# VSF1/foo_dsp_resampler

Measured on AMD Instinct MI355X. Metric: Msamples/s, 44.1k->96k float32 'Best' (input channel-samples), higher is better.
Workload: dtype f64; 1 GPU; BASELINE configs[1]: 44.1k->96k 2ch float32 Best; 256 independent 2-channel streams on this GPU, 481689 frames per push, device-resident in/out (RRX_flow_device); streams_per_gpu=256, frames_per_push=481689, channels=2, chain=dft->poly

## Files before the change

### foo_dsp_resampler_amd/csrc/capi.cpp

```cpp
#include "../../include/ratelib_amd.h"

#include "engine.hpp"
#include "finish.hpp"
#include "lpc.hpp"

#include <algorithm>
#include <atomic>
#include <cstdlib>
#include <cstring>
#include <new>
#include <string>
#include <vector>

struct RR_handle_tag {
  rsmp::Engine *eng;
};

namespace {

void (*g_alloc_handler)(void) = nullptr;
int g_initialized = 0;
std::vector<int> g_devices;
std::atomic<unsigned> g_next_device{0};

// ... 167 lines not shown
  }
  if (device < -1) {
    if (handle) *handle = nullptr;
    return RR_INVPARAM;
  }
  return open_common(config, nchannels, nstreams, device, handle, format);
}

int RRX_format(const RR_handle *h) { return h ? h->eng->format() : -1; }

int RRX_push_samples(RR_handle *h, int format, const void *ibuf, size_t in_stride, size_t isamp)
{ return push_host(h, format, ibuf, in_stride, isamp); }

int RRX_pull_samples(RR_handle *h, int format, void *obuf, size_t out_stride, size_t osamp, size_t *ogen)
{ return pull_host(h, format, obuf, out_stride, osamp, ogen); }

int RRX_flow_samples(RR_handle *h, int format, const void *ibuf, size_t in_stride, void *obuf, size_t out_stride, size_t isamp,
                     size_t osamp, size_t *iused, size_t *ogen)
{
  if (h && h->eng->nstreams() == 1) in_stride = isamp, out_stride = osamp;
  return flow_host(h, format, ibuf, in_stride, obuf, out_stride, isamp, osamp, iused, ogen);
}

int RRX_push_device_samples(RR_handle *h, int format, const void *d_ibuf, size_t in_stride, size_t isamp)
{ return push_device(h, format, d_ibuf, in_stride, isamp); }

int RRX_pull_device_samples(RR_handle *h, int format, void *d_obuf, size_t out_stride, size_t osamp, size_t *ogen)
{ return pull_device(h, format, d_obuf, out_stride, osamp, ogen); }

int RRX_flow_device_samples(RR_handle *h, int format, const void *d_ibuf, size_t in_stride, void *d_obuf, size_t out_stride,
                            size_t isamp, size_t osamp, size_t *iused, size_t *ogen)
{ return flow_device(h, format, d_ibuf, in_stride, d_obuf, out_stride, isamp, osamp, iused, ogen); }

int RRX_push_double(RR_handle *h, const double *ibuf, size_t in_stride, size_t isamp)
{ return push_host(h, RRX_FMT_DOUBLE, ibuf, in_stride, isamp); }

int RRX_pull_double(RR_handle *h, double *obuf, size_t out_stride, size_t osamp, size_t *ogen)
{ return pull_host(h, RRX_FMT_DOUBLE, obuf, out_stride, osamp, ogen); }

int RRX_flow_double(RR_handle *h, const double *ibuf, size_t in_stride, double *obuf, size_t out_stride, size_t isamp, size_t osamp,
                    size_t *iused, size_t *ogen)
{
  if (h && h->eng->nstreams() == 1) in_stride = isamp, out_stride = osamp;
  return flow_host(h, RRX_FMT_DOUBLE, ibuf, in_stride, obuf, out_stride, isamp, osamp, iused, ogen);
}

int RRX_push_device_double(RR_handle *h, const double *d_ibuf, size_t in_stride, size_t isamp)
{ return push_device(h, RRX_FMT_DOUBLE, d_ibuf, in_stride, isamp); }

int RRX_pull_device_double(RR_handle *h, double *d_obuf, size_t out_stride, size_t osamp, size_t *ogen)
{ return pull_device(h, RRX_FMT_DOUBLE, d_obuf, out_stride, osamp, ogen); }

int RRX_flow_device_double(RR_handle *h, const double *d_ibuf, size_t in_stride, double *d_obuf, size_t out_stride, size_t isamp,
                           size_t osamp, size_t *iused, size_t *ogen)
{ return flow_device(h, RRX_FMT_DOUBLE, d_ibuf, in_stride, d_obuf, out_stride, isamp, osamp, iused, ogen); }

int RR_push(RR_handle *h, const fb_sample_t *ibuf, size_t isamp) { return push_host(h, RRX_FMT_FLOAT, ibuf, isamp, isamp); }

int RR_pull(RR_handle *h, fb_sample_t *obuf, size_t osamp, size_t *ogen)
{
  const size_t n = h ? (osamp < h->eng->available() ? osamp : h->eng->available()) : 0;
  return pull_host(h, RRX_FMT_FLOAT, obuf, n, osamp, ogen);
}

int RR_flow(RR_handle *h, const fb_sample_t *ibuf, fb_sample_t *obuf, size_t isamp, size_t osamp, size_t *iused, size_t *ogen)
{
  if (h && h->eng->nstreams() != 1) return RR_INVPARAM;
  return flow_host(h, RRX_FMT_FLOAT, ibuf, isamp, obuf, osamp, isamp, osamp, iused, ogen);
}

int RR_drain(RR_handle *h)
{
  if (!h) return RR_NULLHANDLE;
  return guarded(h, [&] { return h->eng->drain(); });
}

void RR_close(RR_handle **h)
{
  if (h == nullptr || *h == nullptr) return;
  delete (*h)->eng;
  delete *h;
  *h = nullptr;
}

const char *RR_strerror(int error)
{
  switch (error) {
    case RR_OK: return "OK";
    case RR_ENOMEM: return "Not enough memory";
    case RR_INTERNAL: return "Internal error";
    case RR_NULLHANDLE: return "NULL handle";
    case RR_RATEERROR: return "Error in rate() functions";
    case RR_EXTUNINIT: return "Externals not initialized";
    default: return "Other error";
  }
}

int RRX_push_device(RR_handle *h, const fb_sample_t *d_ibuf, size_t in_stride, size_t isamp)
{ return push_device(h, RRX_FMT_FLOAT, d_ibuf, in_stride, isamp); }

int RRX_pull_device(RR_handle *h, fb_sample_t *d_obuf, size_t out_stride, size_t osamp, size_t *ogen)
{ return pull_device(h, RRX_FMT_FLOAT, d_obuf, out_stride, osamp, ogen); }

int RRX_flow_device(RR_handle *h, const fb_sample_t *d_ibuf, size_t in_stride, fb_sample_t *d_obuf, size_t out_stride,
                    size_t isamp, size_t osamp, size_t *iused, size_t *ogen)
{ return flow_device(h, RRX_FMT_FLOAT, d_ibuf, in_stride, d_obuf, out_stride, isamp, osamp, iused, ogen); }

int RRX_push_strided(RR_handle *h, const fb_sample_t *ibuf, size_t in_stride, size_t isamp)
{ return push_host(h, RRX_FMT_FLOAT, ibuf, in_stride, isamp); }

int RRX_pull_strided(RR_handle *h, fb_sample_t *obuf, size_t out_stride, size_t osamp, size_t *ogen)
{ return pull_host(h, RRX_FMT_FLOAT, obuf, out_stride, osamp, ogen); }

int RRX_set_stream(RR_handle *h, void *hip_stream)
{
  if (!h) return RR_NULLHANDLE;
  const bool own = hip_stream == RRX_STREAM_OWN;
  return guarded(h, [&] { return h->eng->set_stream(own ? nullptr : static_cast<hipStream_t>(hip_stream), own); });
}

int RRX_sync(RR_handle *h)
{
  if (!h) return RR_NULLHANDLE;
  return guarded(h, [&] { return h->eng->sync(); });
}

int RRX_profile(RR_handle *h, int enable)
{
  if (!h) return RR_NULLHANDLE;
  return guarded(h, [&] { h->eng->set_profiling(enable != 0); return int(RR_OK); });
}

int RRX_profile_read(RR_handle *h, double *hot_ms, long long *hot_launches, double *other_ms, long long *other_launches)
{
  if (!h) return RR_NULLHANDLE;
  return guarded(h, [&] { return h->eng->read_profile(hot_ms, hot_launches, other_ms, other_launches); });
}

int RRX_profile_report(RR_handle *h, char *buf, size_t cap)
{
  if (!h) return -RR_NULLHANDLE;
  if (!buf || !cap) return -RR_INVPARAM;
  std::string s;
  int rc = guarded(h, [&] { return h->eng->read_profile_json(s); });
  if (rc) return -rc;
  size_t n = s.size() < cap - 1 ? s.size() : cap - 1;
  std::memcpy(buf, s.data(), n);
  buf[n] = 0;
  return int(n);
}

void RRX_debug_fail_alloc(int nth) { rsmp::Engine::fail_alloc_after(nth); }

long long RRX_debug_tile_walk(const RRX_walk_geom *g, int k, long long *head, int *slots, size_t cap)
{
  if (!rsmp::knobs().test_hooks || !g || !head || (cap && !slots) || k < 0) return -1;
  if (g->polyL < 1 || g->step < 1 || g->V < 1 || g->n < 1 || g->KS < 1 || g->nsub < 0 || (g->nsub > 0 && g->Vs < 1)) return -1;
  rsmp::FusedPrepArgs pa;
  pa.b_offset = g->b_offset;
  pa.B0 = g->B0;
  pa.at0 = g->at0;
  pa.V = g->V;
  pa.polyL = g->polyL;
  pa.step = g->step;
  pa.n = g->n;
  pa.nblocks = k + 1;
  pa.two_round = g->two_round;
  pa.KS = g->KS;
  pa.qb_max = g->qb_max;
  pa.qb_min = g->qb_min;
  pa.ra_end = g->ra_end;
  pa.rb_start = g->rb_start;
  pa.clip_lo = 0;
  pa.clip_hi = 0x7fffffffffffffffLL;
  pa.nsub = g->nsub;
  pa.Vs = g->Vs;
  return (long long)rsmp::fused_walk_enumerate(pa, k, head, slots, cap);
}

int RRX_lpc_extrapolate_device(int device, void *hip_stream, fb_sample_t *d_data, size_t stream_stride, int nstreams, size_t data_len,
                               int nch, int lpc_order, size_t extra_bkwd, size_t extra_fwd)
{
  if (!d_data || nstreams < 1 || nch < 1 || lpc_order < 1 || lpc_order > rsmp::kLpcMaxOrder || data_len <= size_t(lpc_order)) return RR_INVPARAM;
  if (nstreams > 1 && stream_stride < extra_bkwd + data_len + extra_fwd) return RR_INVPARAM;
  if (device < -1 || (long long)nstreams * nch > 0x7fffffffLL) return RR_INVPARAM;
  if (!g_initialized) return RR_EXTUNINIT;
  if (!extra_bkwd && !extra_fwd) return RR_OK;
  if (device >= 0) {
    int n = 0;
    if (hipGetDeviceCount(&n) != hipSuccess || n < 1) return RR_EXTUNINIT;
    if (device >= n) return RR_INVPARAM;
  }
  if (!rsmp::device_is_gfx950(device)) return RR_EXTUNINIT;
  rsmp::DeviceScope on(device);
  if (!on.ok()) return RR_INTERNAL;
  const hipError_t e = rsmp::launch_lpc_extrapolate(static_cast<hipStream_t>(hip_stream), d_data, stream_stride, nstreams, data_len,
                                                    nch, lpc_order, extra_bkwd, extra_fwd);
  return e == hipSuccess ? RR_OK : RR_INTERNAL;
}

namespace {

int finish_args(int src_format, const void *src, size_t src_stride, int dst_format, void *dst, size_t dst_stride, int nstreams,
                size_t frames, int nch, const double *gain, int dither, unsigned long long seed, unsigned long long first_frame,
                double *peak, unsigned long long *clipped, rsmp::FinishArgs &a)
{
  if (!src || nstreams < 1 || nch < 1) return RR_INVPARAM;
  if (src_format != RRX_FMT_FLOAT && src_format != RRX_FMT_DOUBLE) return RR_INVPARAM;
  if (dst && dst_format != RRX_FMT_S16 && dst_format != RRX_FMT_S24_3 && dst_format != RRX_FMT_S32) return RR_INVPARAM;
  if (nstreams > 1 && (src_stride < frames || (dst && dst_stride < frames))) return RR_INVPARAM;
  if (!dst && !peak && !clipped) return RR_INVPARAM;
  if (first_frame + frames < first_frame) return RR_INVPARAM;
  const size_t most = (~size_t(0) >> 4) / size_t(nch);
  if (frames > most) return RR_INVPARAM;
  if (nstreams > 1 && (src_stride > most / size_t(nstreams) || (dst && dst_stride > most / size_t(nstreams)))) return RR_INVPARAM;
  a.src = src;
  a.dst = dst;
  a.gain = gain;
  a.peak = peak;
  a.clipped = clipped;
  a.src_stride = nstreams > 1 ? (unsigned long long)src_stride * nch : 0;
  a.dst_stride = nstreams > 1 ? (unsigned long long)dst_stride * nch : 0;
  a.n = (unsigned long long)frames * nch;
  a.seed = seed;
  a.first_frame = first_frame;
  a.nstreams = nstreams;
  a.nch = nch;
  a.src_double = src_format == RRX_FMT_DOUBLE;
  a.bits = !dst ? 31 : dst_format == RRX_FMT_S16 ? 15 : dst_format == RRX_FMT_S24_3 ? 23 : 31;
  a.dither = dither != 0;
  return RR_OK;
}

}

int RRX_finish_device(int device, void *hip_stream, int src_format, const void *d_src, size_t src_stride, int dst_format, void *d_dst,
                      size_t dst_stride, int nstreams, size_t frames, int nch, const double *d_gain, int dither, unsigned long long seed,
                      unsigned long long first_frame, double *d_peak, unsigned long long *d_clipped)
{
  rsmp::FinishArgs a;
  const int rc = finish_args(src_format, d_src, src_stride, dst_format, d_dst, dst_stride, nstreams, frames, nch, d_gain, dither, seed,
                             first_frame, d_peak, d_clipped, a);
  if (rc != RR_OK) return rc;
  if (device < -1) return RR_INVPARAM;
  if (!g_initialized) return RR_EXTUNINIT;
  if (!frames) return RR_OK;
  if (device >= 0) {
    int n = 0;
    if (hipGetDeviceCount(&n) != hipSuccess || n < 1) return RR_EXTUNINIT;
    if (device >= n) return RR_INVPARAM;
  }
  if (!rsmp::device_is_gfx950(device)) return RR_EXTUNINIT;
  rsmp::DeviceScope on(device);
  if (!on.ok()) return RR_INTERNAL;
  return rsmp::launch_finish(static_cast<hipStream_t>(hip_stream), a) == hipSuccess ? RR_OK : RR_INTERNAL;
}

int RRX_debug_finish_host(int src_format, const void *src, size_t src_stride, int dst_format, void *dst, size_t dst_stride, int nstreams,
                          size_t frames, int nch, const double *gain, int dither, unsigned long long seed, unsigned long long first_frame,
                          double *peak, unsigned long long *clipped)
{
  if (!rsmp::knobs().test_hooks) return -1;
  rsmp::FinishArgs a;
  const int rc = finish_args(src_format, src, src_stride, dst_format, dst, dst_stride, nstreams, frames, nch, gain, dither, seed,
                             first_frame, peak, clipped, a);
  if (rc != RR_OK) return rc;
  if (frames) rsmp::finish_host(a);
  return RR_OK;
}

int RRX_edge_geometry(size_t in_rate, size_t out_rate, size_t *n_add, size_t *n_drop, size_t *prime_len, size_t *inbuf)
{
  if (!in_rate || !out_rate || !n_add || !n_drop || !prime_len || !inbuf) return RR_INVPARAM;
  size_t a = in_rate, b = out_rate;
  while (b) { const size_t c = a % b; a = b; b = c; }
  const size_t v = a, r1 = in_rate / v, r2 = out_rate / v, z = r1 > r2 ? r1 : r2;
  size_t n = (v + 20 - 1) / 20;
  if (z * n > 8192) n = 8192 / z;
  if (n < 1) n = 1;
  *n_add = r1 * n;
  *n_drop = r2 * n;
  const size_t prime = std::min<size_t>(std::max<size_t>(in_rate / 20, 1024), 16384);
  *prime_len = std::max<size_t>(prime, 2 * rsmp::kLpcMaxOrder + 1);
  *inbuf = std::min<size_t>(std::max<size_t>(in_rate / 10, 2048), 65536);
  return RR_OK;
}

size_t RRX_isamp_max(const RR_handle *h) { return h ? h->eng->isamp_max() : 0; }
size_t RRX_available(const RR_handle *h) { return h ? h->eng->available() : 0; }
int RRX_channels(const RR_handle *h) { return h ? h->eng->nch() : 0; }
int RRX_streams(const RR_handle *h) { return h ? h->eng->nstreams() : 0; }

int RRX_describe_plan(const RR_config *config, char *buf, size_t cap)
{
  if (!config || !buf || !cap) return -RR_INVPARAM;
  rsmp::ChainPlan plan;
  int rc = rsmp::make_plan(to_config(config), plan);
  if (rc) return -rc;
  std::string s = plan.describe();
  size_t n = s.size() < cap - 1 ? s.size() : cap - 1;
  std::memcpy(buf, s.data(), n);
  buf[n] = 0;
  return int(n);
}

int RRX_describe_dispatch(const RR_config *config, int nchannels, char *buf, size_t cap)
{
  if (!config || !buf || !cap || nchannels < 1) return -RR_INVPARAM;
  rsmp::ChainPlan plan;
  int rc = rsmp::make_plan(to_config(config), plan);
  if (rc) return -rc;
  int nsub = 0, vs = 0;
  const bool sub = !plan.stages.empty() && rsmp::split_geometry(plan, nchannels, 0, nsub, vs);
  std::string s = "{\"sub_blocked\": ";
  s += sub ? "true" : "false";
  if (sub) {
    const rsmp::DftFilter &f = plan.dft[plan.stages[0].filt];
    const int V = f.N - (f.num_taps - 1), Pref = f.N / 2;
    const bool two = nsub == 1 && vs > rsmp::kSplitVsMax;
    char tmp[256];
    snprintf(tmp, sizeof tmp, ", \"two_round\": %s, \"nsub\": %d, \"Vs\": %d, \"V\": %d, \"taps\": %d, \"N\": %d, \"Pref\": %d, \"sub_blocks\": [",
             two ? "true" : "false", nsub, vs, V, f.num_taps, f.N, Pref);
    s += tmp;
    for (int i = 0; i < nsub; ++i) {
      const rsmp::SubBlock sb = rsmp::sub_block(i, V, vs, Pref);
      snprintf(tmp, sizeof tmp, "%s{\"off\": %d, \"len\": %d, \"win\": %d, \"shift\": %d}", i ? ", " : "", sb.off, sb.len, sb.win, sb.shift);
      s += tmp;
    }
    s += "]";
  }
// ... 22 lines not shown
```

### foo_dsp_resampler_amd/csrc/engine.cpp

```cpp
#include "engine.hpp"
#include <cstdio>

#include "design.hpp"

#include <algorithm>
#include <atomic>
#include <climits>
#include <cmath>
#include <cstdint>
#include <cstdlib>
#include <cstring>
#include <new>

namespace rsmp {

namespace {

bool pow2_ge2(int x) { return x >= 2 && !(x & (x - 1)); }
bool fdomain_up(int L) { return pow2_ge2(L) && L <= 4; }
int ilog2(long long v) { int l = 0; while ((1LL << l) < v) ++l; return l; }
long long next_pow2(long long v) { long long p = 1; while (p < v) p <<= 1; return p; }

#define HIP_TRY(expr)                                  \
  do {                                                 \
// ... 246 lines not shown
  if (Pref == 4096) {
    if (fused_split_two_supported(V, f.num_taps, mg.KS, mg.qb_max - mg.qb_min) && V >= 2 * p.n) {
      nsub = 1;
      vs = V;
      return true;
    }
  }
  const int vmax = std::min(kSplitVsMax, (2 * 4096 - (f.num_taps - 1)) & ~1);
  if (vmax < 1024) return false;
  const int n_ = (V + vmax - 1) / vmax, v_ = (((V + n_ - 1) / n_) + 1) & ~1;
  if ((n_ - 1) * v_ >= V) return false;
  for (int k = 0; k < n_; ++k) {
    const SubBlock sb = sub_block(k, V, v_, Pref);
    if ((sb.len & 1) || sb.len < 2 * p.n || 2 * sb.shift + sb.len + (f.num_taps - 1) > 8192) return false;
  }
  nsub = n_;
  vs = v_;
  return true;
}

int Engine::init(const Config &cfg, int nch, int nstreams)
{
  int rc = make_plan(cfg, plan_);
  if (rc) return rc;
  nch_ = nch;
  S_ = nstreams;
  C_ = nch * nstreams;

  if (!device_is_gfx950(device_)) return kUninit;
  if ((rc = init_streams()) != kOk) return rc;
  const Knobs &kn = knobs();
  no_side_ = kn.no_side;
  if (kn.stamps) {
    ALLOC_TRY(&stamps_, 16 * sizeof(unsigned long long));
    HIP_TRY(hipMemset(stamps_, 0, 16 * sizeof(unsigned long long)));
  }
  const int ns = int(plan_.stages.size());
  book_.wr.assign(ns + 1, 0);
  book_.rd.assign(ns + 1, 0);
  book_.st.assign(ns, Book::St());
  rings_.assign(ns + 1, Ring());
  big_.assign(ns, BigDft());
  fuse_.assign(ns, Fuse());
  polymf_.assign(ns, PolyMf());
  for (int i = 0; i <= ns; ++i) rings_[i].frames = (i == 0 || i == ns);
  for (int i = 0; i < ns; ++i) {
    const StageSpec &sp = plan_.stages[i];
    book_.wr[i] = sp.preload;
    if (sp.kind == StageKind::Dft) {
      book_.st[i].remL = sp.remL0;
      if ((rc = init_dft_stage(i)) != kOk) return rc;
    } else if (sp.kind == StageKind::Poly) {
      book_.st[i].at = sp.order == 0 ? (sp.at0 >> 32) : sp.at0;
      if (!d_poly_ && (rc = upload(plan_.poly_table, &d_poly_)) != kOk) return rc;
    }
  }
  size_t fused_slab_cap = 0;
  for (int i = 0; i + 1 < ns; ++i)
    if ((rc = init_fused_pair(i, fused_slab_cap)) != kOk) return rc;
  for (int i = 0; i < ns; ++i)
    if ((rc = init_polymf(i)) != kOk) return rc;
  size_slabs(fused_slab_cap);
  for (int i = 0; i <= ns; ++i)
    if ((rc = ensure_ring(i, std::max<long long>(book_.wr[i], 1))) != kOk) return rc;
  HIP_TRY(hipStreamSynchronize(stream_));
  return kOk;
}

int Engine::init_streams()
{
  HIP_TRY(hipStreamCreateWithFlags(&own_, hipStreamNonBlocking));
  stream_ = own_;
  HIP_TRY(hipEventCreateWithFlags(&ev_switch_, hipEventDisableTiming));
  HIP_TRY(hipStreamCreateWithFlags(&side_, hipStreamNonBlocking));
  HIP_TRY(hipEventCreateWithFlags(&ev_fused_, hipEventDisableTiming));
  HIP_TRY(hipEventCreateWithFlags(&ev_seam_[0], hipEventDisableTiming));
  HIP_TRY(hipEventCreateWithFlags(&ev_seam_[1], hipEventDisableTiming));
  return kOk;
}

int Engine::init_dft_stage(int i)
{
  const StageSpec &sp = plan_.stages[i];
  const DftFilter &f = plan_.dft[sp.filt];
  const int Ng = f.N;
  const int log2n = ilog2(Ng);
  const int log2p = fdomain_up(sp.L) ? log2n - ilog2(sp.L) : log2n;
  const int log2nd = sp.step < 0 ? log2n + sp.step : log2n;
  int sub_n = 0, sub_v = 0;
  const bool sub = split_geometry(i, sub_n, sub_v);
  const bool big = log2n > 14 && !sub;
  if (!sub && (big ? !big_dft_supported(log2n, log2p, log2nd) : !dft_shape_supported(log2n, log2p, log2nd))) return kInvParam;
  int rc;
  if (!d_G_[sp.filt] && (rc = upload(component_spectra(f, Ng, 1, sp.L), &d_G_[sp.filt])) != kOk) return rc;
  if (!big && !d_Gr_[sp.filt] && sp.step == 1 && fdomain_up(sp.L) && dftx_supported(log2n, log2p, log2nd) &&
      (rc = upload(component_spectra(f, Ng, sp.L, sp.L), &d_Gr_[sp.filt])) != kOk)
    return rc;
  if (!big) return sub || (twiddles(log2p) && twiddles(log2nd)) ? kOk : kNoMem;
  BigDft &bg = big_[i];
  bg.on = true;
  if (!twiddles(log2p - 4) || !twiddles(log2nd - 4)) return kNoMem;
  std::vector<double2> tw(Ng);
  for (int j = 0; j < Ng; ++j) {
    const long double th = 2.0L * 3.14159265358979323846264338327950288L * (long double)j / (long double)Ng;
    tw[j] = make_double2((double)cosl(th), (double)sinl(th));
  }
  if ((rc = upload(tw, &bg.twN)) != kOk) return rc;
  const int npairs = pair_count(C_, pair_nchs());
  bg.ws_items = int(std::max<long long>(1, std::min<long long>((256LL << 20) / (16LL * Ng), std::max(4 * npairs, 16))));
  ALLOC_TRY(&bg.w1, size_t(bg.ws_items) * (size_t(1) << log2p) * sizeof(double2));
  ALLOC_TRY(&bg.w2, size_t(bg.ws_items) * (size_t(1) << log2nd) * sizeof(double2));
  return kOk;
}

int Engine::init_fused_pair(int i, size_t &slab_cap)
{
  const Knobs &kn = knobs();
  const StageSpec &d = plan_.stages[i], &p = plan_.stages[i + 1];
  if (d.kind != StageKind::Dft || p.kind != StageKind::Poly || p.order != 0 || d.step != 1) return kOk;
  if (!(d.L == 1 || (pow2_ge2(d.L) && d.L <= 4))) return kOk;
  const DftFilter &f = plan_.dft[d.filt];
  const int log2n = ilog2(f.N), log2p = log2n - (d.L == 1 ? 0 : ilog2(d.L));
  const int G = 2, pstep = int(p.step64 >> 32), at0 = int(p.at0 >> 32);
  int dmax = 0;
  const int NG = (p.L + G - 1) / G;
  for (int m = 0; m < NG; ++m) {
    const long long a0 = at0 + (long long)(G * m) * pstep, a1 = at0 + (long long)std::min(G * m + G - 1, p.L - 1) * pstep;
    dmax = std::max(dmax, int(a1 / p.L - a0 / p.L));
  }
  const int max_seam = int(((long long)(p.n - 1) * p.L + pstep - 1) / pstep) + 1;
  int split_nsub = 0, split_vs = 0;
  split_geometry(i, split_nsub, split_vs);
  const bool split = split_nsub > 0;
  const int threads = split ? 256 : f.N / 16;
  if (!split && (NG > threads || !fused_shape_supported(log2n, log2p, p.n, p.n + dmax, max_seam))) return kOk;
  if (kn.no_fuse) return kOk;
  Fuse &fu = fuse_[i];
  fu.on = true;
  fu.nsub = split_nsub;
  fu.Vs = split_vs;
  int rc;
  if (split) {
    if (!twiddles(12)) return kNoMem;
    if ((rc = upload(component_spectra(f, 8192, 2, d.L), &fu.Gs)) != kOk) return rc;
  }
  fu.span = p.n + dmax;
  fu.NG = NG;
  fu.KC = split ? 1 : threads / NG;
  fu.blk_cap = 64;
  while (fu.blk_cap < kFusedMaxBlocks && double(C_ + 1) * double(4 * fu.blk_cap) * 512 <= kn.seam_ring_mb * 1048576.0) fu.blk_cap *= 2;
  while (fu.blk_cap < 8 * split_nsub) fu.blk_cap *= 2;
  fu.slots = 2 * fu.blk_cap;
  ALLOC_TRY(&fu.blk_dev, size_t(2 * fu.blk_cap) * sizeof(FusedBlock));
  const size_t bytes = size_t(C_ + 1) * fu.slots * 2 * 32 * sizeof(double);
  ALLOC_TRY(&fu.seam, bytes);
  HIP_TRY(hipMemset(fu.seam, 0, bytes));
  const int V = f.N - (f.num_taps - 1);
  const int Kmax = int(((long long)V * p.L / pstep + p.L - 1) / p.L) + 2;
  fu.kper = (Kmax + fu.KC - 1) / fu.KC;
  if (!split && (rc = upload(vector_tiles(p, G, NG, fu.KC, threads, plan_.poly_table), &fu.cft)) != kOk) return rc;
  const MfGeom mg = mf_geom(p);
  bool lanes_spread = true;
  if (kn.spread_vector)
    for (int j1 = 0; j1 < 4; ++j1)
      for (int j2 = j1 + 1; j2 < 4; ++j2)
        if (((j2 - j1) * pstep) % 16 == 0) lanes_spread = false;
  const bool rounds_ok = (mg.qb_max - mg.qb_min) + 4 * mg.KS + 4 <= (kFusedSA - kFusedSB0) * 256 + 32 && Kmax <= 32 && p.L >= 64 && lanes_spread;
  if (split || (!kn.no_mfma && fused_mfma_supported(log2n, log2p, mg.KS) && rounds_ok)) {
    const MfOperands op = mf_operands(mg, p, plan_.poly_table);
    if ((rc = upload(op.cfm, &fu.cfm)) != kOk || (rc = upload(op.cfm2, &fu.cfm2)) != kOk || (rc = upload(op.qtab, &fu.qtab)) != kOk)
      return rc;
    fu.NGRP = mg.NGRP;
    fu.KS = mg.KS;
    fu.qb_max = mg.qb_max;
    fu.qb_min = mg.qb_min;
  }
  const size_t per_launch = size_t(fu.blk_cap / std::max(1, fu.nsub) - 2) * size_t((V - d.remL0 + d.L - 1) / d.L);
  double ahead = 1;
  for (int k = 0; k < i; ++k) ahead *= plan_.stages[k].kind == StageKind::Half ? 0.5 : plan_.stages[k].out_in_ratio;
  const size_t cap = size_t(double(per_launch) / std::max(ahead, 1e-9));
  slab_cap = slab_cap ? std::min(slab_cap, cap) : cap;
  return kOk;
}

int Engine::init_polymf(int i)
{
  const Knobs &kn = knobs();
  const StageSpec &p = plan_.stages[i];
  if (p.kind != StageKind::Poly || p.order != 0 || (i > 0 && fuse_[i - 1].on) || p.L < 64) return kOk;
  if (kn.no_mfma || kn.no_polymf) return kOk;
  const int pstep = int(p.step64 >> 32);
  const MfGeom mg = mf_geom(p);
  if (!polymf_supported(mg.KS)) return kOk;
  int Vt = 2048;
  while (Vt > 256 && ((long long)Vt * p.L / pstep + p.L - 1) / p.L + 2 > 30) Vt -= 256;
  if (((long long)Vt * p.L / pstep + p.L - 1) / p.L + 2 > 30) return kOk;
  const MfOperands op = mf_operands(mg, p, plan_.poly_table);
  PolyMf &pm = polymf_[i];
  int rc;
  if ((rc = upload(op.cfm, &pm.cfm)) != kOk || (rc = upload(op.qtab, &pm.qtab)) != kOk) return rc;
  pm.KS = mg.KS;
  pm.NGRP = mg.NGRP;
  pm.Vt = Vt;
  pm.blk_cap = 4096;
  ALLOC_TRY(&pm.blk, size_t(pm.blk_cap) * sizeof(FusedBlock));
  return kOk;
}

void Engine::size_slabs(size_t fused_slab_cap)
{
  const int ns = int(plan_.stages.size());
  double bytes_per_in_frame = 0, rate = 1;
  for (int i = 0; i < ns; ++i) {
    const StageSpec &sp = plan_.stages[i];
    if (sp.kind == StageKind::Dft) rate *= sp.step > 0 ? double(sp.L) / sp.step : double(sp.L) / double(1 << -sp.step);
    else if (sp.kind == StageKind::Poly) rate *= sp.out_in_ratio;
    else rate *= 0.5;
    if (i + 1 < ns && !fuse_[i].on) bytes_per_in_frame += rate * 8.0 * C_;
  }
  const double budget = knobs().slab_mb * 1024 * 1024;
  slab_frames_ = bytes_per_in_frame > 0 ? size_t(budget / bytes_per_in_frame) : plan_.isamp_max;
  slab_frames_ = std::max<size_t>(slab_frames_, 8192);
  slab_frames_ = std::min<size_t>(slab_frames_, std::max<size_t>(plan_.isamp_max, 1));
  if (fused_slab_cap) slab_frames_ = std::max<size_t>(1024, std::min(slab_frames_, fused_slab_cap));
}

void Engine::set_profiling(bool on)
{
  profiling_ = on;
  for (ProfRec &r : prof_) {
    (void)hipEventDestroy(r.e0);
    (void)hipEventDestroy(r.e1);
  }
  prof_.clear();
}

int Engine::prof_begin(bool hot, const char *name)
{
  if (!profiling_) return -1;
  ProfRec r;
  r.hot = hot;
  r.name = name;
  if (hipEventCreate(&r.e0) != hipSuccess || hipEventCreate(&r.e1) != hipSuccess) return -1;
  (void)hipEventRecord(r.e0, stream_);
  prof_.push_back(r);
  return int(prof_.size()) - 1;
}

void Engine::prof_end(int idx)
{
  if (idx >= 0) (void)hipEventRecord(prof_[idx].e1, stream_);
}

int Engine::read_profile(double *hot_ms, long long *hot_launches, double *other_ms, long long *other_launches)
{
  HIP_TRY(hipStreamSynchronize(stream_));
  double h = 0, o = 0;
  long long hn = 0, on = 0;
  for (ProfRec &r : prof_) {
    float ms = 0;
    if (hipEventElapsedTime(&ms, r.e0, r.e1) == hipSuccess) {
      if (r.hot) { h += ms; ++hn; } else { o += ms; ++on; }
    }
    (void)hipEventDestroy(r.e0);
    (void)hipEventDestroy(r.e1);
  }
  prof_.clear();
  if (hot_ms) *hot_ms = h;
  if (hot_launches) *hot_launches = hn;
  if (other_ms) *other_ms = o;
  if (other_launches) *other_launches = on;
  return kOk;
}

int Engine::read_profile_json(std::string &out)
{
  HIP_TRY(hipStreamSynchronize(stream_));
  struct Agg { const char *name; bool hot; long long n; double ms; };
  std::vector<Agg> agg;
  for (ProfRec &r : prof_) {
    float ms = 0;
    if (hipEventElapsedTime(&ms, r.e0, r.e1) == hipSuccess) {
      Agg *a = nullptr;
      for (Agg &x : agg)
        if (std::strcmp(x.name, r.name) == 0 && x.hot == r.hot) a = &x;
      if (!a) {
        agg.push_back(Agg{r.name, r.hot, 0, 0.0});
        a = &agg.back();
      }
      a->n += 1;
      a->ms += ms;
    }
    (void)hipEventDestroy(r.e0);
    (void)hipEventDestroy(r.e1);
  }
  prof_.clear();
  out = "[";
  char buf[64];
  for (size_t i = 0; i < agg.size(); ++i) {
    out += i ? ", {" : "{";
    out += "\"kernel\": \"";
    out += agg[i].name;
    snprintf(buf, sizeof buf, "\", \"hot\": %d, \"launches\": %lld, \"ms\": %.6f}", agg[i].hot ? 1 : 0, agg[i].n, agg[i].ms);
    out += buf;
  }
  out += "]";
  return kOk;
}

int Engine::join_side()
{
  if (!side_pending_) return kOk;
  HIP_TRY(hipStreamWaitEvent(stream_, ev_seam_[(seam_launches_ - 1) & 1], 0));
  side_pending_ = false;
  return kOk;
}

int Engine::pinned_reserve(Pinned &b, size_t bytes)
{
  if (!b.done) HIP_TRY(hipEventCreateWithFlags(&b.done, hipEventDisableTiming));
  if (b.bytes >= bytes) return kOk;
  if (b.p) {
    HIP_TRY(hipStreamSynchronize(stream_));
    (void)hipHostFree(b.p);
  }
  b.p = nullptr;
  b.bytes = 0;
  size_t want = 16384;
  while (want < bytes) want <<= 1;
  void *p = nullptr;
  if (hipHostMalloc(&p, want, hipHostMallocDefault) != hipSuccess) {
    (void)hipGetLastError();
    return kNoMem;
  }
  b.p = p;
  b.bytes = want;
  return kOk;
}

void Engine::pinned_free(Pinned &b)
{
  if (b.p) (void)hipHostFree(b.p);
  if (b.done) (void)hipEventDestroy(b.done);
  b = Pinned();
}

void Engine::free_garbage()
{
  for (void *p : garbage_) (void)hipFree(p);
  garbage_.clear();
}

Engine::~Engine()
{
  DeviceScope on(device_);
  (void)hipStreamSynchronize(stream_);
  if (own_ && own_ != stream_) (void)hipStreamSynchronize(own_);
  if (side_) (void)hipStreamSynchronize(side_);
  free_garbage();
  for (Ring &r : rings_) if (r.buf) (void)hipFree(r.buf);
  for (double2 *&g : d_G_) if (g) (void)hipFree(g);
  for (double2 *&g : d_Gr_) if (g) (void)hipFree(g);
  if (d_poly_) (void)hipFree(d_poly_);
  for (double2 *&t : d_tw_) if (t) (void)hipFree(t);
  for (double2 *&t : d_tw8_) if (t) (void)hipFree(t);
  set_profiling(false);
  if (d_stage_) (void)hipFree(d_stage_);
  pinned_free(pin_in_[0]);
  pinned_free(pin_in_[1]);
  pinned_free(pin_out_);
  pinned_free(pin_mir_);
  if (stamps_) {
    unsigned long long h[16] = {};
    if (hipMemcpy(h, stamps_, sizeof(h), hipMemcpyDeviceToHost) == hipSuccess && h[7])
      fprintf(stderr, "RSMP_STAMPS workgroups %llu  avg cycles: load %.0f  fwd %.0f  mul %.0f  inv %.0f  cf+smp %.0f  polyA %.0f  poly(B) %.0f  total %.0f\n",
              h[7], double(h[0]) / h[7], double(h[1]) / h[7], double(h[2]) / h[7], double(h[3]) / h[7], double(h[4]) / h[7],
              double(h[6]) / h[7], double(h[5]) / h[7], double(h[0] + h[1] + h[2] + h[3] + h[4] + h[5] + h[6]) / h[7]);
    (void)hipFree(stamps_);
  }
  for (Fuse &f : fuse_) {
    if (f.seam) (void)hipFree(f.seam);
    if (f.cft) (void)hipFree(f.cft);
    if (f.cfm) (void)hipFree(f.cfm);
    if (f.qtab) (void)hipFree(f.qtab);
    if (f.cfm2) (void)hipFree(f.cfm2);
    if (f.Gs) (void)hipFree(f.Gs);
    if (f.blk_dev) (void)hipFree(f.blk_dev);
  }
  for (BigDft &b : big_) {
    if (b.twN) (void)hipFree(b.twN);
    if (b.w1) (void)hipFree(b.w1);
    if (b.w2) (void)hipFree(b.w2);
  }
  for (PolyMf &m : polymf_) {
    if (m.cfm) (void)hipFree(m.cfm);
    if (m.qtab) (void)hipFree(m.qtab);
    if (m.blk) (void)hipFree(m.blk);
  }
  if (side_) (void)hipStreamDestroy(side_);
  if (ev_fused_) (void)hipEventDestroy(ev_fused_);
  for (hipEvent_t &e : ev_seam_) if (e) (void)hipEventDestroy(e);
  if (ev_switch_) (void)hipEventDestroy(ev_switch_);
  if (own_) (void)hipStreamDestroy(own_);
}

int Engine::set_stream(hipStream_t s, bool own)
{
  hipStream_t next = own ? own_ : s;
  if (next == stream_) return kOk;
  { int rcj = join_side(); if (rcj) return rcj; }
  HIP_TRY(hipEventRecord(ev_switch_, stream_));
  HIP_TRY(hipStreamWaitEvent(next, ev_switch_, 0));
  stream_ = next;
  return kOk;
}

int Engine::sync()
{
  HIP_TRY(hipStreamSynchronize(stream_));
  free_garbage();
  return kOk;
}

AnyView Engine::view(int f, const ExtIn *ein, const ExtOut *eout) const
{
  const Ring &r = rings_[f];
  AnyView v = {};
  if (!r.frames) {
    v.kind = kRingF64;
    v.d.ring = static_cast<double *>(r.buf);
    v.d.mask = r.cap - 1;
    v.d.chan_stride = r.cap;
    return v;
  }
  v.kind = fk_;
  v.f.ring = r.buf;
  v.f.ring_mask = r.cap - 1;
  v.f.ring_stream_stride = r.cap * nch_;
  v.f.nch = nch_;
  if (ein && ein->ptr) {
    v.f.ext = const_cast<void *>(ein->ptr);
    v.f.ext_begin = ein->begin;
    v.f.ext_end = ein->end;
    v.f.ext_stream_stride = ein->stride_elems;
  } else if (eout && eout->ptr) {
    v.f.ext = eout->ptr;
    v.f.ext_begin = eout->begin;
    v.f.ext_end = eout->end;
    v.f.ext_stream_stride = eout->stride_elems;
  }
  return v;
}

int Engine::ensure_ring(int f, long long live_needed)
{
  Ring &r = rings_[f];
  if (r.buf && r.cap >= live_needed) return kOk;
  { int rcj = join_side(); if (rcj) return rcj; }
  const long long cap = next_pow2(std::max<long long>({live_needed, r.cap * 2, 4096}));
  const size_t bytes = r.frames ? size_t(cap) * nch_ * S_ * size_t(eb_) : size_t(cap) * C_ * sizeof(double);
  void *nb = nullptr;
  ALLOC_TRY(&nb, bytes);
  HIP_TRY(hipMemsetAsync(nb, 0, bytes, stream_));
  if (r.buf) {
    Ring old = r;
    r.buf = nb;
    r.cap = cap;
    const long long a0 = book_.rd[f], a1 = book_.wr[f];
    const AnyView dst = view(f);
    AnyView src = dst;
    if (r.frames) {
      src.f.ring = old.buf;
      src.f.ring_mask = old.cap - 1;
      src.f.ring_stream_stride = old.cap * nch_;
    } else {
      src.d.ring = static_cast<double *>(old.buf);
      src.d.mask = old.cap - 1;
      src.d.chan_stride = old.cap;
    }
    HIP_TRY(launch_copy(src, dst, a0, a1, C_, stream_));
    garbage_.push_back(old.buf);
  } else {
    r.buf = nb;
    r.cap = cap;
  }
  return kOk;
}

void Engine::note_input(Book &b, size_t n) const
{
  b.samples_in += n;
  while (b.samples_in > plan_.cfg.in_rate && b.samples_out > plan_.cfg.out_rate) {
    b.samples_in -= plan_.cfg.in_rate;
    b.samples_out -= plan_.cfg.out_rate;
  }
}

#define RSMP_STAGE_LOCALS(ps, i)                                                                                   \
  Book &b = (ps).b;                                                                                                \
  const bool launch = (ps).launch;                                                                                 \
  const ExtIn &ein = (ps).ein;                                                                                     \
  const ExtOut &eout = (ps).eout;                                                                                  \
  const int ns = int(plan_.stages.size());                                                                         \
  const StageSpec &sp = plan_.stages[i];                                                                           \
  Book::St &st = b.st[i];                                                                                          \
  long long &rd = b.rd[i];                                                                                         \
  long long &wro = b.wr[(i) + 1];                                                                                  \
  const long long occ = b.wr[i] - rd;                                                                              \
                                              \
  const bool src_frames = (i) == 0, dst_frames = (i) + 1 == ns;                                                    \
  const long long rd_before = rd, wro_before = wro;                                                                \
  const long long out_offset = (i) + 1 < ns ? plan_.stages[(i) + 1].preload : -b.trimmed;                          \
  Pending &pend = (ps).pend;                                                                                       \
                                      \
  auto dst_need = [&](long long wr_after) {                                                                        \
    if (dst_frames && eout.ptr) return std::max<long long>(0, wr_after - std::max(eout.end, b.rd[(i) + 1]));      \
    return wr_after - b.rd[(i) + 1];                                                                               \
  };                                                                                                               \
  (void)rd_before; (void)wro_before; (void)out_offset; (void)occ; (void)src_frames; (void)dst_frames;             \
  (void)launch; (void)ein; (void)pend; (void)st; (void)dst_need

int Engine::advance(Book &b, size_t n_new, bool launch, const ExtIn &ein, const ExtOut &eout, bool more_slabs)
{
  note_input(b, n_new);
  b.wr[0] += (long long)n_new;
  Pass ps{b, launch, ein, eout, more_slabs, Pending()};
  for (int i = 0; i < int(plan_.stages.size()); ++i) {
    const StageKind kind = plan_.stages[i].kind;
    const int rc = kind == StageKind::Dft ? advance_dft(ps, i) : kind == StageKind::Poly ? advance_poly(ps, i) : advance_half(ps, i);
    if (rc) return rc;
  }
  return kOk;
}

int Engine::advance_dft(Pass &ps, int i)
{
  RSMP_STAGE_LOCALS(ps, i);
  DftArgs &pend_args = pend.args;
  int &pend_log2n = pend.log2n, &pend_log2p = pend.log2p;
  const DftFilter &f = plan_.dft[sp.filt];
// ... 39 lines not shown
    if (!sub && !big && log2p >= 6 && log2p <= 13 && !a.tw_fwd8) return kNoMem;
    a.tw_inv8 = (!sub && !big && log2nd >= 6 && log2nd <= 12) ? twiddles8(log2nd) : nullptr;
    if (!sub && !big && log2nd >= 6 && log2nd <= 12 && !a.tw_inv8) return kNoMem;
    a.B0 = B0;
    a.out_offset = out_offset;
    a.nblocks = nblocks;
    a.C = C_;
    a.L = L;
    a.c0 = pow2_ge2(L) ? 0 : sp.remL0;
    a.V = Vg;
    a.Vout = sp.step < 0 ? Ng - ((((1 << -sp.step) - 1) * Ng + ov) >> -sp.step) : Vg;
    a.q = (Vg - sp.remL0 + L - 1) / L;
    a.M = sp.step > 1 ? sp.step : 1;
    a.hp = 0;
    a.nchs = pair_nchs();
    a.in_limit = 0x7fffffffffffffffLL;
    a.clip_lo = -0x7fffffffffffffffLL;
    a.clip_hi = 0x7fffffffffffffffLL;
    a.nsub = a.Vs = a.Pref = a.two = 0;
    a.Bref0 = 0;
    if (big) {
      const BigDft &bg = big_[i];
      BigDftArgs ba;
      ba.d = a;
      ba.twN = bg.twN;
      ba.w1 = bg.w1;
      ba.w2 = bg.w2;
      ba.log2n = log2n;
      ba.log2mp = log2p - 4;
      ba.log2md = log2nd - 4;
      ba.fdomain_in = (log2p < log2n || L == 1) ? 1 : 0;
      ba.item0 = 0;
      const int pi = prof_begin(true, "rsmp::big_cols_fwd_kernel + big_rows_kernel + big_cols_inv_kernel");
      HIP_TRY(launch_dft_big(view(i, &ein), view(i + 1, nullptr, &eout), ba, bg.ws_items, stream_));
      prof_end(pi);
    } else
    if (fused) {
      pend.B0 = B0;
      pend.nblocks = nblocks;
      pend_args = a;
      pend_log2n = log2n;
      pend_log2p = log2p;
    } else if (a.Gr && sp.step == 1 && fdomain_up(L) && dftx_supported(log2n, log2p, log2nd)) {
      const int pi = prof_begin(true);
      const char *kn = nullptr;
      HIP_TRY(launch_dftx(log2n, view(i, &ein), view(i + 1, nullptr, &eout), a, stream_, &kn));
      prof_name(pi, kn);
      prof_end(pi);
    } else {
    const int pi = prof_begin(true);
    const char *kn = nullptr;
    HIP_TRY(launch_dft(log2n, log2p, log2nd, view(i, &ein), view(i + 1, nullptr, &eout), a, stream_, &kn));
    prof_name(pi, kn);
    prof_end(pi);
    }
  }
  return kOk;
}

int Engine::advance_poly(Pass &ps, int i)
{
  RSMP_STAGE_LOCALS(ps, i);
  const long long num_in = std::max<long long>(0, occ - sp.pre_post);
  long long count = 0, at_end = st.at;
  const long long step = sp.order == 0 ? (sp.step64 >> 32) : sp.step64;
  const long long lim = sp.order == 0 ? num_in * sp.L : (num_in << 32);
  if (st.at < lim) count = (lim - st.at + step - 1) / step;
  at_end = st.at + count * step;
  const bool fused = i > 0 && fuse_[i - 1].on;
  if (launch && fused) {
    if ((count != 0) != (pend.nblocks != 0)) return kInternal;
    if (pend.nblocks) {
      const int rc = launch_fused_pair(ps, i, count, step);
      if (rc) return rc;
    }
  } else if (launch && count && polymf_[i].cfm) {
    const int rc = launch_polymf_stage(ps, i, count, step);
    if (rc) return rc;
  } else if (launch && count) {
    const int rc = launch_poly_stage(ps, i, count, step);
    if (rc) return rc;
  }
  if (sp.order == 0) {
    rd += at_end / sp.L;
    st.at = at_end % sp.L;
  } else {
    rd += at_end >> 32;
    st.at = at_end & 0xffffffffLL;
  }
  wro += count;
  return kOk;
}

int Engine::launch_fused_pair(Pass &ps, int i, long long count, long long step)
{
  RSMP_STAGE_LOCALS(ps, i);
  const bool more_slabs = ps.more_slabs;
  DftArgs &pend_args = pend.args;
  const int pend_log2n = pend.log2n, pend_log2p = pend.log2p;
  int rc = ensure_ring(i + 1, dst_need(wro + count));
  if (rc) return rc;
  const Fuse &fu = fuse_[i - 1];
  FusedArgs fa;
  fa.d = pend_args;
  fa.tab = d_poly_;
  fa.seam = fu.seam;
  fa.cft = fu.cft;
  fa.at0 = sp.at0 >> 32;
  fa.b_offset = sp.preload;
  fa.out_offset2 = out_offset;
  fa.seam_mask = fu.slots - 1;
  fa.n = sp.n;
  fa.polyL = sp.L;
  fa.step = int(step);
  fa.span = fu.span;
  fa.NG = fu.NG;
  fa.KC = fu.KC;
  fa.kper = fu.kper;
  fa.cfm = fu.cfm;
  fa.qtab = fu.qtab;
  fa.cfm2 = fu.cfm2;
  fa.NGRP = fu.NGRP;
  fa.KS = fu.KS;
  fa.stamps = stamps_;
  const bool split = fu.nsub > 0;
  const int ntab = split ? pend.nblocks * fu.nsub : pend.nblocks;
  if (ntab > fu.blk_cap) return kInternal;
  FusedPrepArgs pa;
  pa.b_offset = fa.b_offset;
  pa.B0 = pend.B0;
  pa.at0 = fa.at0;
  pa.V = fa.d.V;
  pa.polyL = sp.L;
  pa.step = int(step);
  pa.n = sp.n;
  pa.nblocks = ntab;
  pa.nsub = fu.nsub;
  pa.Vs = fu.Vs;
  const bool split_two = split && fu.nsub == 1 && fu.Vs > kSplitVsMax;
  pa.two_round = fu.cfm != nullptr && (!split || split_two);
  pa.ra_end = split_two ? kSplitRaEnd : 0;
  pa.rb_start = split_two ? kSplitRbStart : 0;
  pa.KS = fu.KS;
  pa.qb_max = fu.qb_max;
  pa.qb_min = fu.qb_min;
  pa.clip_lo = 0;
  pa.clip_hi = 0x7fffffffffffffffLL;
  if (!split)
    for (int k : {0, pend.nblocks - 1})
      if (fused_block_info(pa, k).K > (fu.cfm ? 32 : fu.KC * fu.kper)) return kInternal;
  const bool seam_on_side = more_slabs && !(profiling_ || !dst_frames || no_side_);
  if (seam_launches_ >= 2) HIP_TRY(hipStreamWaitEvent(stream_, ev_seam_[seam_launches_ & 1], 0));
  FusedBlock *const blk_half = fu.blk_dev + size_t(seam_launches_ & 1) * fu.blk_cap;
  { const int pp = prof_begin(false, "rsmp::fused_prep_kernel"); HIP_TRY(launch_fused_prep(pa, blk_half, stream_)); prof_end(pp); }
  fa.blk = blk_half;
  const long long endnum = (b.wr[i] - sp.n + 1) * sp.L - fa.at0;
  if (wro - out_offset + count != (endnum <= 0 ? 0 : (endnum + step - 1) / step)) return kInternal;
  const bool in_frames = i - 1 == 0;
  int f0 = 0, f1 = 0;
  FastIo io = {};
  io.dio = fk_ - kFramesF32;
  const uintptr_t amask = 2 * uintptr_t(eb_) - 1;
  auto io_in = [&] {
    io.in = ein.ptr;
    io.in_ring = rings_[0].buf;
    io.in_ring_mask = rings_[0].cap - 1;
    io.in_ring_stream_stride = rings_[0].cap * nch_;
    io.in_abs0 = ein.begin;
    io.in_stream_stride = ein.stride_elems;
    io.nch = nch_;
  };
  auto io_out64 = [&] {
    io.out64 = static_cast<double *>(rings_[i + 1].buf);
    io.out64_mask = rings_[i + 1].cap - 1;
    io.out64_chan_stride = rings_[i + 1].cap;
  };
  if (split) {
    if (!in_frames || (nch_ & 1) || !ein.ptr || (ein.stride_elems & 1)) return kInternal;
    io_in();
    io.in_unaligned = (reinterpret_cast<uintptr_t>(ein.ptr) & amask) ? 1 : 0;
    int omode = 1;
    if (!dst_frames)
      io_out64();
    else {
      const bool ext_ok = eout.ptr && !(eout.stride_elems & 1);
      const bool all_inside = ext_ok && wro >= eout.begin && wro + count <= eout.end;
      omode = (all_inside && !(reinterpret_cast<uintptr_t>(eout.ptr) & amask)) ? 0 : 2;
      io.out = ext_ok ? eout.ptr : nullptr;
      io.out_abs0 = ext_ok ? eout.begin : 0;
      io.out_end = ext_ok ? eout.end : 0;
      io.out_stream_stride = ext_ok ? eout.stride_elems : 0;
      io.out_unaligned = (ext_ok && (reinterpret_cast<uintptr_t>(eout.ptr) & amask)) ? 1 : 0;
      io.out_ring = rings_[i + 1].buf;
      io.out_ring_mask = rings_[i + 1].cap - 1;
      io.out_ring_stream_stride = rings_[i + 1].cap * nch_;
      if (eout.ptr && !ext_ok) return kInternal;
      if (omode == 2 && !io.out_ring) return kInternal;
    }
    FusedArgs fr = fa;
    fr.d.G = fu.Gs;
    fr.d.tw_fwd = fr.d.tw_inv = twiddles(12);
    if (!fr.d.tw_fwd) return kNoMem;
    fr.d.nsub = fu.nsub;
    fr.d.Vs = fu.Vs;
    fr.d.two = split_two ? 1 : 0;
    fr.d.Pref = 1 << pend_log2p;
    fr.d.Bref0 = pend.B0;
    fr.d.B0 = pend.B0 * fu.nsub;
    fr.d.nblocks = ntab;
    fa = fr;
    const int pi = prof_begin(true);
    const char *kn = nullptr;
    HIP_TRY(launch_fused_split(omode, fr, io, stream_, &kn));
    prof_name(pi, kn);
    prof_end(pi);
  } else if (fu.cfm && in_frames && dst_frames && !(nch_ & 1) && ein.ptr && eout.ptr && fused_fast_supported(pend_log2n, pend_log2p, fu.KS) &&
             !(reinterpret_cast<uintptr_t>(ein.ptr) & amask) && !(reinterpret_cast<uintptr_t>(eout.ptr) & amask) &&
             !(ein.stride_elems & 1) && !(eout.stride_elems & 1)) {
    const long long P = 1LL << pend_log2p, q = fa.d.q;
    const long long hi = (ein.end - P) >= 0 ? (ein.end - P) / q - pend.B0 + 1 : 0;
    f0 = 0;
    f1 = int(std::min<long long>(pend.nblocks, hi));
    while (f0 < f1) {
      const FusedBlock b0 = fused_block_info(pa, f0), b1 = fused_block_info(pa, f1 - 1);
      if (out_offset + b0.i_lo < eout.begin) { ++f0; continue; }
      if (out_offset + b1.i_lo + b1.cnt > eout.end) { --f1; continue; }
      break;
    }
    if (f0 >= f1) f0 = f1 = 0;
    io_in();
    io.out = eout.ptr;
    io.out_abs0 = eout.begin;
    io.out_stream_stride = eout.stride_elems;
  } else if (fu.cfm && in_frames && !dst_frames && !(nch_ & 1) && ein.ptr && fused_fast_supported(pend_log2n, pend_log2p, fu.KS) &&
             !(reinterpret_cast<uintptr_t>(ein.ptr) & amask) && !(ein.stride_elems & 1)) {
    const long long P = 1LL << pend_log2p, q = fa.d.q;
    const long long hi = (ein.end - P) >= 0 ? (ein.end - P) / q - pend.B0 + 1 : 0;
    f0 = 0;
    f1 = int(std::max<long long>(0, std::min<long long>(pend.nblocks, hi)));
    io_in();
    io_out64();
  }
  auto launch_range = [&](int b0, int b1, bool fast) -> int {
    if (b0 >= b1) return kOk;
    FusedArgs fr = fa;
    fr.d.B0 = fa.d.B0 + b0;
    fr.d.nblocks = b1 - b0;
    fr.blk = fa.blk + b0;
    const int pi = prof_begin(true);
    const char *kn = nullptr;
    if (fast) HIP_TRY(launch_fused_fast(pend_log2p, fr, io, stream_, &kn));
    else
      HIP_TRY(launch_fused(pend_log2n, pend_log2p, view(i - 1, &ein), view(i + 1, nullptr, &eout), fr, stream_, &kn));
    prof_name(pi, kn);
    prof_end(pi);
    return kOk;
  };
  if (!split) {
    { int rl = launch_range(0, f0, false); if (rl) return rl; }
    { int rl = launch_range(f0, f1, true); if (rl) return rl; }
    { int rl = launch_range(f1, pend.nblocks, false); if (rl) return rl; }
  }
  if (!seam_on_side) {
    { int rcj = join_side(); if (rcj) return rcj; }
    const int ps = prof_begin(false, "rsmp::seam_kernel");
    HIP_TRY(launch_seam(view(i + 1, nullptr, &eout), fa, stream_));
    prof_end(ps);
  } else {
    HIP_TRY(hipEventRecord(ev_fused_, stream_));
    HIP_TRY(hipStreamWaitEvent(side_, ev_fused_, 0));
    HIP_TRY(launch_seam(view(i + 1, nullptr, &eout), fa, side_));
    HIP_TRY(hipEventRecord(ev_seam_[seam_launches_ & 1], side_));
    ++seam_launches_;
    side_pending_ = true;
  }
  return kOk;
}

int Engine::launch_polymf_stage(Pass &ps, int i, long long count, long long step)
{
  RSMP_STAGE_LOCALS(ps, i);
  int rc = ensure_ring(i + 1, dst_need(wro + count));
  if (rc) return rc;
  const PolyMf &pm = polymf_[i];
  const long long at0 = sp.at0 >> 32, i_begin = wro_before - out_offset, i_end = i_begin + count;
  const long long q_first = (at0 + i_begin * step) / sp.L, q_last = (at0 + (i_end - 1) * step) / sp.L;
  for (long long t0 = q_first / pm.Vt, t_end = q_last / pm.Vt + 1; t0 < t_end; t0 += pm.blk_cap) {
    FusedPrepArgs pa;
    pa.b_offset = 0;
    pa.B0 = t0;
    pa.at0 = at0;
    pa.V = pm.Vt;
    pa.polyL = sp.L;
    pa.step = int(step);
    pa.n = 1;
    pa.nblocks = int(std::min<long long>(pm.blk_cap, t_end - t0));
    pa.two_round = 0;
    pa.ra_end = pa.rb_start = 0;
    pa.nsub = pa.Vs = 0;
    pa.KS = pm.KS;
    pa.qb_max = 0;
    pa.qb_min = 0;
    pa.clip_lo = i_begin;
    pa.clip_hi = i_end;
    for (int k : {0, pa.nblocks - 1})
      if (fused_block_info(pa, k).K > 32) return kInternal;
    { const int pp = prof_begin(false, "rsmp::fused_prep_kernel"); HIP_TRY(launch_fused_prep(pa, pm.blk, stream_)); prof_end(pp); }
    PolyMfArgs a;
    a.cfm = pm.cfm;
    a.qtab = pm.qtab;
    a.blk = pm.blk;
    a.B0 = t0;
    a.at0 = at0;
    a.out_offset = out_offset;
    a.in_limit = b.wr[i];
    a.nblocks = pa.nblocks;
    a.C = C_;
    a.Vt = pm.Vt;
    a.n = sp.n;
    a.polyL = sp.L;
    a.step = int(step);
    a.NGRP = pm.NGRP;
    a.nchs = pair_nchs();
    const int pi = prof_begin(false);
    const char *kn = nullptr;
    HIP_TRY(launch_polymf(pm.KS, view(i, &ein), view(i + 1, nullptr, &eout), a, stream_, &kn));
    prof_name(pi, kn);
    prof_end(pi);
  }
  return kOk;
}

int Engine::launch_poly_stage(Pass &ps, int i, long long count, long long step)
{
  RSMP_STAGE_LOCALS(ps, i);
  int rc = ensure_ring(i + 1, dst_need(wro + count));
  if (rc) return rc;
  PolyArgs a;
  a.tab = d_poly_;
  a.rd = rd_before;
  a.at = st.at;
  a.step = step;
  a.out_abs = wro_before;
  a.count = count;
  a.C = C_;
  a.n = sp.n;
  a.L = sp.L;
  a.phase_bits = sp.phase_bits;
  const double in_per_out = sp.order == 0 ? double(step) / sp.L : double(step) / 4294967296.0;
  const size_t tab_bytes = sp.order == 0 ? size_t(sp.L) * sp.n * 8 : 0;
  const bool tab_lds = sp.order == 0 && tab_bytes <= 40 * 1024;
  const double lds_for_window = tab_lds ? double(64 * 1024 - 16) - double(tab_bytes) : 48.0 * 1024;
  int tile = 2048;
  while (tile > 256 && ((tile * in_per_out + sp.n + 4) * 8 > lds_for_window ||
                        (sp.order == 0 && double(tile + 256) * double(step) >= 2147483648.0)))
    tile >>= 1;
  if (sp.order == 0 && double(tile + 256) * double(step) >= 2147483648.0) return kInternal;
  a.tile = tile;
  a.win = (int(tile * in_per_out) + sp.n + 4 + 1) & ~1;
  a.tab_lds = tab_lds;
  a.coop = sp.order >= 1 && sp.n % 8 == 0 && !knobs().no_polycoop;
  a.shared_rows = 0;
  if (sp.order >= 1 && sp.n <= 32 && !knobs().no_polyi) {
    const double wl = 128 * in_per_out + sp.n + 4;
    if ((128.0 * sp.n + 16.0 * (wl + 1)) * 8 <= 150.0 * 1024) {
      a.shared_rows = 1;
      a.tile = 128;
      a.win = int(wl) | 1;
    }
  }
  const int pi = prof_begin(false);
  const char *kn = nullptr;
  HIP_TRY(launch_poly(sp.order, view(i, &ein), view(i + 1, nullptr, &eout), a, stream_, &kn));
  prof_name(pi, kn);
  prof_end(pi);
  return kOk;
}

int Engine::advance_half(Pass &ps, int i)
{
  RSMP_STAGE_LOCALS(ps, i);
  const long long avail = std::max<long long>(0, occ - sp.pre_post);
  const long long num_out = (avail + 1) / 2;
  if (launch && num_out) {
    int rc = ensure_ring(i + 1, dst_need(wro + num_out));
    if (rc) return rc;
    HalfArgs a;
    a.rd = rd_before;
    a.out_abs = wro_before;
    a.count = num_out;
    a.C = C_;
    a.ncoef = sp.hb_n;
    a.pre = sp.pre;
    for (int k = 0; k < 13; ++k) a.coef[k] = k < sp.hb_n ? sp.hb[k] : 0.0;
    const int pi = prof_begin(false);
    const char *kn = nullptr;
    HIP_TRY(launch_half(view(i, &ein), view(i + 1, nullptr, &eout), a, stream_, &kn));
    prof_name(pi, kn);
    prof_end(pi);
  }
  if (2 * num_out <= occ) rd += 2 * num_out;
// ... 336 lines not shown
```

### foo_dsp_resampler_amd/csrc/engine.hpp

```cpp
#pragma once
#include "kernels.hpp"
#include "plan.hpp"

#include <hip/hip_runtime.h>
#include <cstddef>
#include <cstdint>
#include <string>
#include <vector>

namespace rsmp {

enum { kOk = 0, kNoMem = 1, kInternal = 2, kNullHandle = 3, kRateError = 4, kUninit = 5, kInvParam = 6 };

struct Book {
  std::vector<long long> wr, rd;
  struct St { long long B = 0; int remL = 0, remM = 0; long long at = 0; };
  std::vector<St> st;
  size_t samples_in = 0, samples_out = 0;
  long long trimmed = 0;
};

bool split_geometry(const ChainPlan &plan, int nch, int i, int &nsub, int &vs);

class DeviceScope {
public:
  explicit DeviceScope(int device)
  {
    if (hipGetDevice(&prev_) != hipSuccess) prev_ = -1;
    if (device >= 0 && device != prev_) ok_ = hipSetDevice(device) == hipSuccess, switched_ = ok_;
  }
  ~DeviceScope() { if (switched_ && prev_ >= 0) (void)hipSetDevice(prev_); }
  DeviceScope(const DeviceScope &) = delete;
  DeviceScope &operator=(const DeviceScope &) = delete;
  bool ok() const { return ok_; }
private:
  int prev_ = -1;
  bool ok_ = true, switched_ = false;
};

class Engine {
public:
  static int create(const Config &cfg, int nch, int nstreams, int device, Engine **out, int fmt = 0);
  ~Engine();

  int device() const { return device_; }
  int format() const { return fmt_; }

  const ChainPlan &plan() const { return plan_; }
  int nch() const { return nch_; }
  int nstreams() const { return S_; }
  int pair_nchs() const { return (S_ > 1 && (nch_ & 1)) ? nch_ : 0; }
  size_t isamp_max() const { return plan_.isamp_max; }
  size_t available() const { return size_t(book_.wr.back() - book_.rd.back()); }

  int set_stream(hipStream_t s, bool own = false);
  hipStream_t stream() const { return stream_; }
  int sync();
  static void fail_alloc_after(int n);

  int push_host(const void *ibuf, size_t stream_stride, size_t isamp);
  int pull_host(void *obuf, size_t stream_stride, size_t osamp, size_t *ogen);
  int flow_host(const void *ibuf, size_t in_stride, void *obuf, size_t out_stride, size_t isamp, size_t osamp, size_t *iused,
                size_t *ogen);
  int push_device(const void *ibuf, size_t stream_stride, size_t isamp);
  int pull_device(void *obuf, size_t stream_stride, size_t osamp, size_t *ogen);
  int flow_device(const void *ibuf, size_t in_stride, void *obuf, size_t out_stride, size_t isamp, size_t osamp, size_t *iused,
                  size_t *ogen);
  int drain();

  void set_profiling(bool on);
  int read_profile(double *hot_ms, long long *hot_launches, double *other_ms, long long *other_launches);
  int read_profile_json(std::string &out);

private:
  Engine() = default;
  int init(const Config &cfg, int nch, int nstreams);
  int init_streams();
  int init_dft_stage(int i);
  int init_fused_pair(int i, size_t &slab_cap);
  int init_polymf(int i);
  void size_slabs(size_t fused_slab_cap);
  int fmt_ = 0, eb_ = 4, fk_ = kFramesF32;
  size_t frame_bytes() const { return size_t(nch_) * size_t(eb_); }
  static const void *at_bytes(const void *p, size_t bytes) { return static_cast<const char *>(p) + bytes; }
  static void *at_bytes(void *p, size_t bytes) { return static_cast<char *>(p) + bytes; }

  struct Ring {
    void *buf = nullptr;
    long long cap = 0;
    bool frames = false;
  };
  struct ExtIn { const void *ptr = nullptr; long long begin = 0, end = 0, stride_elems = 0; };
  struct ExtOut { void *ptr = nullptr; long long begin = 0, end = 0, stride_elems = 0; };

  int feed(const void *d_in, size_t stride_frames, size_t isamp, void *d_out, size_t out_stride, size_t out_cap,
           size_t *direct_out, bool keep_direct = false);
  int feed_impl(const void *d_in, size_t stride_frames, size_t isamp, void *d_out, size_t out_stride, size_t out_cap,
                size_t *direct_out, bool keep_direct);
  int advance(Book &b, size_t n_new, bool launch, const ExtIn &ein, const ExtOut &eout, bool more_slabs = false);
  struct Pending { long long B0 = 0; int nblocks = 0; DftArgs args = {}; int log2n = 0, log2p = 0; };
  struct Pass { Book &b; bool launch; const ExtIn &ein; const ExtOut &eout; bool more_slabs; Pending pend; };
  int advance_dft(Pass &ps, int i);
  int advance_poly(Pass &ps, int i);
  int advance_half(Pass &ps, int i);
  int launch_fused_pair(Pass &ps, int i, long long count, long long step);
  bool split_geometry(int i, int &nsub, int &vs) const;
  int launch_polymf_stage(Pass &ps, int i, long long count, long long step);
  int launch_poly_stage(Pass &ps, int i, long long count, long long step);
  int ensure_ring(int f, long long live_needed);
  int copy_out(void *dst, size_t stride_frames, size_t frames, bool to_host);
  AnyView view(int f, const ExtIn *ein = nullptr, const ExtOut *eout = nullptr) const;
  void note_input(Book &b, size_t n) const;
  template <class T> int upload(const std::vector<T> &src, T **dst);
  const double2 *twiddles(int log2m);
  const double2 *twiddles8(int log2m);
  void free_garbage();

  ChainPlan plan_;
  int nch_ = 0, S_ = 0, C_ = 0;
  int device_ = 0;
  hipStream_t stream_ = nullptr;
  hipStream_t own_ = nullptr;
  hipEvent_t ev_switch_ = nullptr;
  bool poisoned_ = false;
  int fail(int rc) { if (rc != kOk) poisoned_ = true; return rc; }
  int dev_alloc(void **p, size_t bytes);
  hipStream_t side_ = nullptr;
  hipEvent_t ev_fused_ = nullptr, ev_seam_[2] = {nullptr, nullptr};
  long long seam_launches_ = 0;
  bool side_pending_ = false;
  int join_side();
  Book book_;
  std::vector<Ring> rings_;
  std::vector<void *> garbage_;
  double2 *d_G_[2] = {nullptr, nullptr};
  double2 *d_Gr_[2] = {nullptr, nullptr};
  double *d_poly_ = nullptr;
  double2 *d_tw_[20] = {};
  double2 *d_tw8_[20] = {};
  struct BigDft { bool on = false; double2 *twN = nullptr, *w1 = nullptr, *w2 = nullptr; int ws_items = 0; };
  std::vector<BigDft> big_;
  struct Fuse { bool on = false; int span = 0, NG = 0, KC = 0, kper = 0; double *seam = nullptr; double *cft = nullptr; int slots = 0;
                double *cfm = nullptr; int NGRP = 0, KS = 0, qb_max = 0, qb_min = 0; int *qtab = nullptr; double2 *cfm2 = nullptr;
                FusedBlock *blk_dev = nullptr; int blk_cap = 0;
                int nsub = 0, Vs = 0; double2 *Gs = nullptr; };
  std::vector<Fuse> fuse_;
  struct PolyMf { double *cfm = nullptr; int *qtab = nullptr; FusedBlock *blk = nullptr; int KS = 0, NGRP = 0, Vt = 0, blk_cap = 0; };
  std::vector<PolyMf> polymf_;
  struct ProfRec { hipEvent_t e0, e1; bool hot; const char *name; };
  std::vector<ProfRec> prof_;
  bool profiling_ = false;
  int prof_begin(bool hot, const char *name = "");
  void prof_name(int idx, const char *name) { if (idx >= 0 && name) prof_[idx].name = name; }
  void prof_end(int idx);
  bool no_side_ = false;
  unsigned long long *stamps_ = nullptr;
  void *d_stage_ = nullptr;
  size_t stage_bytes_ = 0;
  struct Pinned { void *p = nullptr; size_t bytes = 0; hipEvent_t done = nullptr; bool pending = false; };
  Pinned pin_in_[2], pin_out_;
  int pin_k_ = 0;
  static constexpr size_t kPinnedMaxBytes = size_t(64) << 20;
  static constexpr size_t kZeroCopyMaxBytes = size_t(1) << 20;
  Pinned pin_mir_;
  long long mir_begin_ = 0, mir_end_ = 0;
  size_t mir_stride_ = 0;
  int spill_mirror();
  int pinned_reserve(Pinned &b, size_t bytes);
  void pinned_free(Pinned &b);
  size_t slab_frames_ = 0;
};

bool device_is_gfx950(int device = -1);

}
```

### foo_dsp_resampler_amd/csrc/fused.hip

```cpp
#include "fft_device.hpp"
#include "fifo_device.hpp"
#include "kernels.hpp"

#include <algorithm>
#include <type_traits>
#include <atomic>
#include <cstdlib>
#include <cstdio>


namespace rsmp {

constexpr int kPad = 32;
constexpr int kSpanMax = 32;
constexpr int kSA = kFusedSA, kSB0 = kFusedSB0;

template <int LOG2N, int LOG2P, int G, int SPAN, bool MF>
__global__ __launch_bounds__((1 << LOG2N) / 16, MF ? kFusedWaves : 2) void fused_kernel(AnyView in, AnyView out, FusedArgs a)
{
  constexpr int N = 1 << LOG2N, P = 1 << LOG2P;
  constexpr int T = N / 16, TF = P / 16;
  extern __shared__ __attribute__((aligned(16))) double lds[];

  const int tid = threadIdx.x;
// ... 335 lines not shown
      const int kr0 = kc * kper, kr1 = min(kr0 + kper, fb.K);

      bool ofast = false;
      float *obase = nullptr;
      int ostride = 1;
      const PairSpan o64 = out.kind >= kFramesF64 ? pair_span(out, pair, hasb, a.out_offset2 + fb.i_lo, fb.cnt, ca)
                                                    : PairSpan{0, nullptr, 1, nullptr, nullptr, hasb};
      {
        const long long o0 = a.out_offset2 + fb.i_lo, o1 = o0 + fb.cnt;
        if (out.kind == kFramesF32 && hasb && !(out.f.nch & 1)) {
          const int hp = out.f.nch >> 1, strm = pair / hp, pin = pair - strm * hp;
          ostride = hp;
          if (out.f.ext && o0 >= out.f.ext_begin && o1 <= out.f.ext_end) {
            obase = static_cast<float *>(out.f.ext) + strm * out.f.ext_stream_stride + (o0 - out.f.ext_begin) * out.f.nch + 2 * pin;
            ofast = true;
          } else if ((!out.f.ext || o0 >= out.f.ext_end || o1 <= out.f.ext_begin) &&
                     (o0 & out.f.ring_mask) + (o1 - o0) <= out.f.ring_mask + 1) {
            obase = static_cast<float *>(out.f.ring) + strm * out.f.ring_stream_stride + (o0 & out.f.ring_mask) * out.f.nch + 2 * pin;
            ofast = true;
          }
          ofast = ofast && (reinterpret_cast<unsigned long long>(obase) & 7) == 0;
        }
      }

      for (int kr = kr0; kr < kr1; ++kr) {
        const int ib = kr * pl + r0;
        bool ok[G], any = false;
#pragma unroll
        for (int g = 0; g < G; ++g) {
          ok[g] = rv[g] && ib + g >= fb.irel_lo && ib + g < irel_hi;
          any = any || ok[g];
        }
        if (!any) continue;
        const int li = qr0 + kr * step + fb.base_li;
        const double2 *xw = smp + li;
        double accA[G], accB[G];
#pragma unroll
        for (int g = 0; g < G; ++g) accA[g] = accB[g] = 0.0;
#pragma unroll
        for (int mm = 0; mm < SPAN; ++mm) {
          const double2 xv = xw[mm];
#pragma unroll
          for (int g = 0; g < G; ++g) {
            accA[g] = fma(cf[g][mm], xv.x, accA[g]);
            accB[g] = fma(cf[g][mm], xv.y, accB[g]);
          }
        }
        const int orel = ib - fb.irel_lo;
        if (ofast) {
          float2 *o2 = reinterpret_cast<float2 *>(obase) + orel * ostride;
          if (G == 2 && ostride == 1 && ok[0] && ok[1] && (reinterpret_cast<unsigned long long>(o2) & 15) == 0) {
            *reinterpret_cast<float4 *>(o2) = make_float4((float)accA[0], (float)accB[0], (float)accA[1], (float)accB[1]);
          } else {
#pragma unroll
            for (int g = 0; g < G; ++g)
              if (ok[g]) o2[g * ostride] = make_float2((float)accA[g], (float)accB[g]);
          }
        } else if (o64.kind == 3) {
#pragma unroll
          for (int g = 0; g < G; ++g)
            if (ok[g]) o64.d2[(orel + g) * o64.fstride] = make_double2(accA[g], accB[g]);
        } else if (o64.kind >= 4) {
#pragma unroll
          for (int g = 0; g < G; ++g)
            if (ok[g]) o64.puti(orel + g, accA[g], accB[g]);
        } else {
          const ChanRef oa = chan_ref(out, ca), ob = chan_ref(out, hasb ? cb : ca);
          const long long oabs = a.out_offset2 + fb.i_lo + orel;
#pragma unroll
          for (int g = 0; g < G; ++g)
            if (ok[g]) {
              fifo_put(oa, oabs + g, accA[g]);
              if (hasb) fifo_put(ob, oabs + g, accB[g]);
            }
        }
      }
    }
    RSMP_STAMP(5)
    if (stamping && tid == 0) atomicAdd(a.stamps + 7, 1ull);
  }
#undef RSMP_STAMP
}

constexpr int kSeamC = 64, kSeamWin = 2 * 31 + 3, kSeamOut = 64;
__global__ __launch_bounds__(256) void seam_kernel(AnyView out, FusedArgs a)
{
  __shared__ double win[kSeamC][kSeamWin];
  __shared__ double cfs[kSeamOut][32];
  __shared__ int qs[kSeamOut];
  const int bl = blockIdx.x, c0 = blockIdx.y * kSeamC, tid = threadIdx.x;
  const long long B = a.d.B0 + bl;
  const int nm1 = a.n - 1, pl = a.polyL, step = a.step, n = a.n;
  const int nc = min(kSeamC, a.d.C - c0);
  const FusedBlock fb = a.blk[bl];
  const int cnt = min((int)(fb.i_lo - fb.seam_i0), kSeamOut);
  {
    const int k = tid & 63;
    const double *const tails = a.seam + ((long long)((int)((B - 1) & a.seam_mask) * (a.d.C + 1) + c0) * 2 + 1) * 32;
    const double *const heads = a.seam + ((long long)((int)(B & a.seam_mask) * (a.d.C + 1) + c0) * 2) * 32;
    const bool wk = k < 2 * nm1;
    const double *const src = k < nm1 ? tails + k : heads + (min(k, 2 * nm1 - 1) - nm1);
    const bool zero = k < nm1 && B == 0;
    double tw[kSeamC / 4];
#pragma unroll
    for (int i = 0; i < kSeamC / 4; ++i) tw[i] = src[min((tid >> 6) + 4 * i, nc - 1) * 64];
    const int j = min(tid & 31, n - 1);
    double t[kSeamOut / 8];
    int q[kSeamOut / 8];
#pragma unroll
    for (int i = 0; i < kSeamOut / 8; ++i) {
      t[i] = 0.0;
      q[i] = 0;
      if (8 * i < cnt) {
        const int u = min((tid >> 5) + 8 * i, cnt - 1);
        const unsigned tc = (unsigned)fb.seam_ph0 + (unsigned)u * (unsigned)step;
        const unsigned qq = tc / (unsigned)pl, ph = tc - qq * (unsigned)pl;
        q[i] = fb.seam_q0 + (int)qq;
        t[i] = a.tab[(long long)ph * n + j];
      }
    }
    if (wk) {
#pragma unroll
      for (int i = 0; i < kSeamC / 4; ++i) {
        const int cl = (tid >> 6) + 4 * i;
        if (cl < nc) win[cl][k] = zero ? 0.0 : tw[i];
      }
    }
#pragma unroll
    for (int i = 0; i < kSeamOut / 8; ++i) {
      const int u = (tid >> 5) + 8 * i;
      if (u < cnt) {
        if ((tid & 31) < n) cfs[u][j] = t[i];
        if ((tid & 31) == 0) qs[u] = q[i];
      }
    }
  }
  __syncthreads();
  {
    const int cl = tid & 63;
    if (cl < nc) {
      const ChanRef oc = chan_ref(out, c0 + cl);
      for (int u = tid >> 6; u < cnt; u += 4) {
        const double *x = win[cl] + qs[u];
        const double *cf = cfs[u];
        double sum = 0.0;
#pragma unroll 8
        for (int j = 0; j < n; ++j) sum = fma(cf[j], x[j], sum);
        fifo_put(oc, a.out_offset2 + fb.seam_i0 + u, sum);
      }
    }
  }
}

__global__ __launch_bounds__(256) void fused_prep_kernel(FusedPrepArgs p, FusedBlock *out)
{
  const int k = blockIdx.x * 256 + threadIdx.x;
  if (k < p.nblocks) out[k] = fused_block_info(p, k);
}

hipError_t launch_fused_prep(const FusedPrepArgs &p, FusedBlock *out, hipStream_t st)
{
  hipLaunchKernelGGL(fused_prep_kernel, dim3((p.nblocks + 255) / 256), dim3(256), 0, st, p, out);
  return hipGetLastError();
}

template <int LOG2N, int LOG2P, int G, int SPAN, bool MF>
static hipError_t launch_fused_t(const AnyView &in, const AnyView &out, const FusedArgs &a, hipStream_t st)
{
  constexpr int N = 1 << LOG2N;
  const size_t lds_pad = knobs().lds_pad;
  size_t lds_bytes = 8 * size_t(fft_lds_doubles(LOG2N));
  if (MF) {
    lds_bytes = 8 * size_t(fft_lds_doubles_halves(LOG2N));
    if (LOG2P < LOG2N) lds_bytes = std::max(lds_bytes, 8 * size_t(std::max(fft_lds_doubles(LOG2P), fft8_lds_doubles(LOG2P))));
    lds_bytes = std::max(lds_bytes, size_t(kPad + kSA * (N / 16) + kPad) * 16);
  }
  lds_bytes += lds_pad;
  static DynLdsOnce attr;
  static std::atomic<bool> occ_printed{false};
  if (hipError_t e = attr.set(reinterpret_cast<const void *>(&fused_kernel<LOG2N, LOG2P, G, SPAN, MF>), int(lds_bytes)); e != hipSuccess) return e;
  {
    if (knobs().occ && !occ_printed.exchange(true)) {
      int nb = -1;
      hipError_t eo = hipOccupancyMaxActiveBlocksPerMultiprocessor(&nb, reinterpret_cast<const void *>(&fused_kernel<LOG2N, LOG2P, G, SPAN, MF>), N / 16, lds_bytes);
      fprintf(stderr, "RSMP_OCC lds %zu blocks/CU %d (%s)\n", lds_bytes, nb, hipGetErrorString(eo));
    }
  }
  FusedArgs b = a;
  b.d.hp = frame_pairs(in, out, a.d.C);
  b.d.npairs = pair_count(a.d.C, a.d.nchs);
  b.d.pps_magic = pair_magic(a.d.C, a.d.nchs);
  dim3 grid(item_grid(a.d.nblocks, b.d.npairs, b.d.hp)), block(N / 16);
  hipLaunchKernelGGL((fused_kernel<LOG2N, LOG2P, G, SPAN, MF>), grid, block, lds_bytes, st, in, out, b);
  return hipGetLastError();
}

hipError_t launch_seam(const AnyView &out, const FusedArgs &a, hipStream_t st)
{
  dim3 sgrid(a.d.nblocks, (a.d.C + kSeamC - 1) / kSeamC), sblock(256);
  hipLaunchKernelGGL(seam_kernel, sgrid, sblock, 0, st, out, a);
  return hipGetLastError();
}

bool fused_mfma_supported(int log2n, int log2p, int ksteps)
{
  return log2n == 12 && (log2p == 11 || log2p == 12) && (ksteps == 7 || ksteps == 8);
}

bool fused_shape_supported(int log2n, int log2p, int n, int span, int max_seam_outputs)
{
  if (log2n < 11 || log2n > 13) return false;
  if (log2p > log2n || log2p < log2n - 2) return false;
  return n >= 4 && n <= 32 && span <= kSpanMax && max_seam_outputs <= 64;
}

#define RSMP_FUSED_CASE(n, p)                                                     \
  if (log2n == n && log2p == p) {                                                 \
    if (kname) *kname = "rsmp::fused_kernel<" #n ", " #p ", 2, 32, false>";       \
    return launch_fused_t<n, p, 2, kSpanMax, false>(in, out, a, st);              \
  }
#define RSMP_FUSED_EXACT(n, p, sp)                                                \
  if (log2n == n && log2p == p && a.span == sp) {                                 \
    if (kname) *kname = "rsmp::fused_kernel<" #n ", " #p ", 2, " #sp ", false>";  \
    return launch_fused_t<n, p, 2, sp, false>(in, out, a, st);                    \
  }
#define RSMP_FUSED_MF(n, p, ks)                                                   \
  if (log2n == n && log2p == p && a.KS == ks) {                                   \
    if (kname) *kname = "rsmp::fused_kernel<" #n ", " #p ", 2, " #ks ", true>";   \
    return launch_fused_t<n, p, 2, ks, true>(in, out, a, st);                     \
  }

hipError_t launch_fused(int log2n, int log2p, const AnyView &in, const AnyView &out, const FusedArgs &a, hipStream_t st,
                        const char **kname)
{
  if (a.cfm) {
    RSMP_FUSED_MF(12, 11, 7) RSMP_FUSED_MF(12, 12, 7) RSMP_FUSED_MF(12, 11, 8) RSMP_FUSED_MF(12, 12, 8)
    return hipErrorInvalidValue;
  }
  RSMP_FUSED_EXACT(12, 11, 25) RSMP_FUSED_EXACT(12, 11, 26) RSMP_FUSED_EXACT(12, 12, 26) RSMP_FUSED_EXACT(12, 12, 27)
  RSMP_FUSED_CASE(11, 11) RSMP_FUSED_CASE(11, 10) RSMP_FUSED_CASE(11, 9)
  RSMP_FUSED_CASE(12, 12) RSMP_FUSED_CASE(12, 11) RSMP_FUSED_CASE(12, 10)
  RSMP_FUSED_CASE(13, 13) RSMP_FUSED_CASE(13, 12) RSMP_FUSED_CASE(13, 11)
  return hipErrorInvalidValue;
}

}
```

### foo_dsp_resampler_amd/csrc/fused_fast.hip

```cpp
#include "fft_device.hpp"
#include "fifo_device.hpp"
#include "kernels.hpp"

#include <algorithm>
#include <atomic>
#include <cstdlib>
#include <cstdio>
#include <type_traits>

namespace rsmp {

namespace {
typedef unsigned int rsmp_v2u __attribute__((ext_vector_type(2)));
typedef unsigned int rsmp_v4u __attribute__((ext_vector_type(4)));
template <typename E> struct Frame;
template <> struct Frame<float> {
  typedef float2 P;
  static __device__ __forceinline__ double in(float s) { return (double)s; }
  static __device__ __forceinline__ float out(double y) { return (float)y; }
};
template <> struct Frame<double> {
  typedef double2 P;
  static __device__ __forceinline__ double in(double s) { return s; }
  static __device__ __forceinline__ double out(double y) { return y; }
};
template <> struct Frame<short> {
  typedef short2 P;
  static __device__ __forceinline__ double in(short s) { return pcm_in(s); }
  static __device__ __forceinline__ short out(double y) { return pcm_out16(y); }
};
template <> struct Frame<int> {
  typedef int2 P;
  static __device__ __forceinline__ double in(int s) { return pcm_in(s); }
  static __device__ __forceinline__ int out(double y) { return pcm_out32(y); }
};
__device__ __forceinline__ double2 load_g(const double2 *p) { return *p; }
constexpr int kPad = 32;
constexpr int kSA = kFusedSA, kSB0 = kFusedSB0;
}

template <int LOG2P, int KS, bool OUT64, bool SPLIT, bool OGEN, bool TWO = false, typename E = float>
__device__ __forceinline__ void fused_fast_body(const FusedArgs &a, const FastIo &io)
{
  typedef Frame<E> Fr;
  typedef typename Fr::P E2;
  const E *const io_in = static_cast<const E *>(io.in), *const io_in_ring = static_cast<const E *>(io.in_ring);
  E *const io_out = static_cast<E *>(io.out), *const io_out_ring = static_cast<E *>(io.out_ring);
  static_assert(!TWO || SPLIT, "two rounds from registers: sub-blocked form only");
  static_assert(!SPLIT || LOG2P == 12, "sub-blocked form: 4096-point components");
  static_assert(!OGEN || (SPLIT && !OUT64), "generic float output exists for the sub-blocked form only");
  constexpr int LOG2N = 12, N = 1 << LOG2N, P = 1 << LOG2P;
  constexpr int T = N / 16, TF = P / 16;
  extern __shared__ __attribute__((aligned(16))) double lds[];

  const int tid = threadIdx.x;
  const int npairs = a.d.C >> 1;
  int bl, pair;
  if (!item_map(blockIdx.x, a.d.nblocks, npairs, a.d.hp, bl, pair)) return;
  const long long B = a.d.B0 + bl;
  const int hp = io.nch >> 1, strm = pair / hp, pin = pair - strm * hp;
  SubBlock sb = {0, 0, 0, 0};
  long long e0_split = 0;
  if constexpr (SPLIT) {
    const int kr = bl / a.d.nsub;
    sb = sub_block(bl - kr * a.d.nsub, a.d.V, a.d.Vs, a.d.Pref);
    e0_split = (a.d.Bref0 + kr) * a.d.q + sb.win;
  }
  const int V = SPLIT ? sb.len : a.d.V;
  const bool fwd_active = tid < TF;
  const double2 *__restrict__ Gp = a.d.G;
  double2 *smp = reinterpret_cast<double2 *>(lds) + kPad;
  const int nm1 = a.n - 1;

#ifdef RSMP_STAMPS_BUILD
  const bool stamping = a.stamps && (blockIdx.x & 63) == 5;
  unsigned long long tstamp = stamping ? __builtin_readcyclecounter() : 0;
#define RSMP_STAMP(slot)                                          \
  if (stamping) {                                                  \
    const unsigned long long now = __builtin_readcyclecounter();  \
    if (tid == 0) atomicAdd(a.stamps + (slot), now - tstamp);      \
    tstamp = now;                                                  \
  }
#else
#define RSMP_STAMP(slot)
#endif

  constexpr bool FWD8 = LOG2P == LOG2N - 1;
  constexpr int NLD = FWD8 ? 8 : 16, TL = FWD8 ? T : TF;
  c64 v[16];
  c64 u8[8];
  c64 z0[SPLIT ? 16 : 1];
  double2 wf[FWD8 ? fft8_tw_regs(LOG2P) : 1];
  if constexpr (FWD8) fft8_tw_load<LOG2P>(wf, tid, a.d.tw_fwd8);
  {
    const long long e0 = SPLIT ? e0_split : B * a.d.q;
    const bool ld_active = FWD8 || fwd_active;
    if (SPLIT && io.in_unaligned) {
      const E *pe = io_in + strm * io.in_stream_stride + 2 * pin, *pr = io_in_ring + strm * io.in_ring_stream_stride + 2 * pin;
#pragma unroll
      for (int s = 0; s < NLD; ++s) {
        const long long e = e0 + tid + s * TL;
        const E *f = e >= io.in_abs0 ? pe + (e - io.in_abs0) * io.nch : pr + (e & io.in_ring_mask) * io.nch;
        v[s] = {Fr::in(f[0]), Fr::in(f[1])};
      }
    } else
    if (e0 >= io.in_abs0) {
      const E2 *p2 = reinterpret_cast<const E2 *>(io_in + strm * io.in_stream_stride + (e0 - io.in_abs0) * io.nch + 2 * pin);
      if (ld_active) {
#pragma unroll
        for (int s = 0; s < NLD; ++s) {
          const E2 f = p2[(unsigned)((tid + s * TL) * hp)];
          (FWD8 ? u8[s & 7] : v[s]) = {Fr::in(f.x), Fr::in(f.y)};
        }
      }
    } else if (ld_active) {
      const E *pe = io_in + strm * io.in_stream_stride + 2 * pin, *pr = io_in_ring + strm * io.in_ring_stream_stride + 2 * pin;
#pragma unroll
      for (int s = 0; s < NLD; ++s) {
        const long long e = e0 + tid + s * TL;
        const E2 f = *reinterpret_cast<const E2 *>(e >= io.in_abs0 ? pe + (e - io.in_abs0) * io.nch : pr + (e & io.in_ring_mask) * io.nch);
        (FWD8 ? u8[s & 7] : v[s]) = {Fr::in(f.x), Fr::in(f.y)};
      }
    }
  }
  RSMP_STAMP(0)
  if constexpr (FWD8) {
    double2 g[16];
    fft8_regs_pre<LOG2P, -1>(u8, tid, wf, lds, [&](int p) {
      if (p == 1) {
#pragma unroll
        for (int s = 0; s < 16; ++s) g[s] = load_g(Gp + (unsigned)(tid + s * T));
      }
    });
    RSMP_STAMP(1)
#pragma unroll
    for (int s = 0; s < 16; ++s) v[s] = cmul(u8[s & 7], c64{g[s].x, g[s].y});
    __syncthreads();
  } else {
  fft_regs<LOG2P, -1, LOG2P == LOG2N ? 2 : 0, kPfFwd>(v, tid, fwd_active, a.d.tw_fwd, lds);
  RSMP_STAMP(1)
  if constexpr (LOG2P < LOG2N) {
    double2 g[16];
#pragma unroll
    for (int s = 0; s < 16; ++s) g[s] = load_g(Gp + tid + s * T);
    double2 *l2 = reinterpret_cast<double2 *>(lds);
    if (fwd_active) {
#pragma unroll
      for (int u = 0; u < 8; ++u) l2[tid + u * TF] = make_double2(v[2 * u + 1].x, v[2 * u + 1].y);
    }
    __syncthreads();
    c64 z[8];
    if (fwd_active) {
#pragma unroll
      for (int u = 0; u < 8; ++u) z[u] = v[2 * u];
    } else {
#pragma unroll
      for (int u = 0; u < 8; ++u) {
        const double2 q = l2[tid - TF + u * TF];
        z[u] = {q.x, q.y};
      }
    }
#pragma unroll
    for (int s = 0; s < 16; ++s) v[s] = cmul(z[s & 7], c64{g[s].x, g[s].y});
    __syncthreads();
  } else if constexpr (SPLIT) {
    c64 xs[16];
#pragma unroll
    for (int s = 0; s < 16; ++s) {
      xs[s] = v[s];
      const double2 g = load_g(Gp + tid + s * T);
      v[s] = cmul(xs[s], c64{g.x, g.y});
    }
    fft_regs<LOG2N, +1, 2, kPfInv>(v, tid, true, a.d.tw_inv, lds);
    double2 g1[16];
#pragma unroll
    for (int s = 0; s < 16; ++s) g1[s] = load_g(Gp + N + tid + s * T);
#pragma unroll
    for (int s = 0; s < 16; ++s) {
      z0[s] = v[s];
      v[s] = cmul(xs[s], c64{g1[s].x, g1[s].y});
    }
    __syncthreads();
    fft_regs<LOG2N, +1, 2, kPfInv>(v, tid, true, a.d.tw_inv, lds);
  } else {
#pragma unroll
    for (int s = 0; s < 16; ++s) {
      const double2 g = load_g(Gp + tid + s * T);
      v[s] = cmul(v[s], c64{g.x, g.y});
    }
  }
  }
  RSMP_STAMP(2)
  if constexpr (!SPLIT) fft_regs<LOG2N, +1, 2, kPfInv>(v, tid, true, a.d.tw_inv, lds);
  RSMP_STAMP(3)

  const int ca = 2 * pair, cb = ca + 1;
  {
    const int slot = (int)(B & a.seam_mask);
    double *seamA = a.seam + ((long long)(slot * (a.d.C + 1) + ca) * 2) * 32;
    double *seamB = a.seam + ((long long)(slot * (a.d.C + 1) + cb) * 2) * 32;
    if constexpr (SPLIT && TWO) {
      __syncthreads();
#pragma unroll
      for (int s = 0; s <= kSplitSA; ++s) {
        const int n = 2 * (tid + s * T);
        if (n < V && (s < kSplitSA || tid < kPad / 2)) {
          smp[n] = make_double2(z0[s].x, z0[s].y);
          smp[n + 1] = make_double2(v[s].x, v[s].y);
        }
      }
      if (tid < kPad) {
        smp[tid - kPad] = make_double2(0.0, 0.0);
        if (V < kSplitRaEnd + kPad) smp[V + tid] = make_double2(0.0, 0.0);
      }
      (void)seamA; (void)seamB;
    } else if constexpr (SPLIT) {
      __syncthreads();
#pragma unroll
      for (int s = 0; s < 16; ++s) {
        const int n = 2 * (tid + s * T - sb.shift);
        if (n >= 0 && n < V) {
          smp[n] = make_double2(z0[s].x, z0[s].y);
          smp[n + 1] = make_double2(v[s].x, v[s].y);
        }
      }
      if (tid < kPad) {
        smp[tid - kPad] = make_double2(0.0, 0.0);
        smp[V + tid] = make_double2(0.0, 0.0);
      }
      (void)seamA; (void)seamB;
    } else {
#pragma unroll
    for (int s = 0; s <= kSA; ++s) {
      const int n = tid + s * T;
      const bool whole = (s + 1) * T <= V;
      if (s < kSA ? (whole || n < V) : (tid < kPad && n < V)) smp[n] = make_double2(v[s].x, v[s].y);
    }
    if (tid < nm1) {
      seamA[tid] = v[0].x;
      seamB[tid] = v[0].y;
    }
    if (tid < kPad) {
      smp[tid - kPad] = make_double2(0.0, 0.0);
      if (V < kSA * T + kPad) smp[V + tid] = make_double2(0.0, 0.0);
    }
    }
  }
  __syncthreads();
  if constexpr (SPLIT) {
    if (tid < nm1) {
      const int slot = (int)(B & a.seam_mask);
      const double2 t = smp[tid];
      a.seam[((long long)(slot * (a.d.C + 1) + ca) * 2) * 32 + tid] = t.x;
      a.seam[((long long)(slot * (a.d.C + 1) + cb) * 2) * 32 + tid] = t.y;
    }
  }
  const int tail0 = V - nm1;
  auto store_tail = [&](const double2 *img, int n0) {
    if (tid < nm1) {
      const int slot = (int)(B & a.seam_mask);
      const double2 t = img[tail0 + tid - n0];
      a.seam[((long long)(slot * (a.d.C + 1) + ca) * 2 + 1) * 32 + tid] = t.x;
      a.seam[((long long)(slot * (a.d.C + 1) + cb) * 2 + 1) * 32 + tid] = t.y;
    }
  };
  const bool tail_in_b = TWO ? tail0 >= kSplitRbStart : (!SPLIT && tail0 >= kSB0 * T);
  if (!tail_in_b) store_tail(smp, 0);
  RSMP_STAMP(4)

  const FusedBlock fb = a.blk[bl];
  const int lane = tid & 63, wave = __builtin_amdgcn_readfirstlane(tid >> 6);
  const int hi = lane >> 4, bq = (lane >> 2) & 3, jq = lane & 3;
  const int pl = a.polyL, step = a.step;
  const int frame_bytes = io.nch * (int)sizeof(E);
  char *const obytes = (OUT64 || OGEN) ? nullptr
                            : reinterpret_cast<char *>(io_out + strm * io.out_stream_stride + (a.out_offset2 + fb.i_lo - io.out_abs0) * io.nch + 2 * pin);
  const long long oabs0 = a.out_offset2 + fb.i_lo;
  E *const oext = OGEN ? io_out + strm * io.out_stream_stride + 2 * pin : nullptr;
  E *const oring = OGEN ? io_out_ring + strm * io.out_ring_stream_stride + 2 * pin : nullptr;
  const unsigned o64 = OUT64 ? (unsigned)((a.out_offset2 + fb.i_lo) & io.out64_mask) : 0u;
  const unsigned m64 = (unsigned)io.out64_mask;
  __amdgpu_buffer_rsrc_t orsrcA, orsrcB;
  if constexpr (OUT64) {
    double *ra = io.out64 + (long long)(2 * pair) * io.out64_chan_stride;
    orsrcA = __builtin_amdgcn_make_buffer_rsrc(ra, 0, (int)((io.out64_mask + 1) * 8), 0x00020000);
    orsrcB = __builtin_amdgcn_make_buffer_rsrc(ra + io.out64_chan_stride, 0, (int)((io.out64_mask + 1) * 8), 0x00020000);
  }
  const int rloc = 4 * bq + hi;
  const int ngrp = a.NGRP;
  const double2 *const cfm_lane = a.cfm2 + lane;
  const int *const qtab_lane = a.qtab + bq;

  const FusedWalk fw = fused_walk(fb, ngrp);
  auto poly_round = [&](int kb, int ke, const double2 *xs, int li_lo, int li_hi) {
    if (ke <= kb) return;
    const WalkRound wr = walk_round(fw, fb.K, kb, ke, ngrp);
    const int t0 = (wr.nt * wave) >> 2, t1 = (wr.nt * (wave + 1)) >> 2;
    if (t0 >= t1) return;
    int g, pc;
    walk_seek(wr, t0, g, pc);
    g = __builtin_amdgcn_readfirstlane(g);
    int p0 = __builtin_amdgcn_readfirstlane(walk_p0(fw, g));
    pc = __builtin_amdgcn_readfirstlane(4 * pc + p0);
    int pend = __builtin_amdgcn_readfirstlane(p0 + 4 * walk_ncs(fw, fb.K, kb, ke, g));
    const int lane_li = walk_lane_li(fb, kb, hi, jq, step);
    const int lane_ib = walk_lane_ib(fb, kb, jq, rloc, pl);
    const int cnt = walk_round_cnt(fb, fw, ke, pl);
    const __amdgpu_buffer_rsrc_t orsrc =
        __builtin_amdgcn_make_buffer_rsrc(obytes, 0, (!OUT64 && !OGEN && cnt > 0) ? (cnt - 1) * frame_bytes + 2 * (int)sizeof(E) : 0, 0x00020000);
    const int lane_off0 = __mul24(lane_ib, frame_bytes);
    const bool lane_dead_last = 16 * (ngrp - 1) + rloc >= pl;

    double cc[KS], cn[KS];
    double qcd = 0.0, qnd = 0.0;
    int qci = 0, qni = 0;
    auto load_tile = [&](int gg, double (&c_)[KS], double &qd_, int &qi_) {
      constexpr int KSP = (KS + 1) / 2;
      const double2 *cp = cfm_lane + gg * (KSP * 64);
#pragma unroll
      for (int s2 = 0; s2 < KSP; ++s2) {
        const double2 d = cp[s2 * 64];
        c_[2 * s2] = d.x;
        if (2 * s2 + 1 < KS) c_[2 * s2 + 1] = d.y;
        else qd_ = d.y;
      }
      if (!(KS & 1)) qi_ = qtab_lane[gg * 4];
    };
    auto qof = [&](double qd_, int qi_) { return (KS & 1) ? (int)qd_ : qi_; };
    load_tile(g, cc, qcd, qci);
    load_tile(min(g + 1, ngrp - 1), cn, qnd, qni);

    double2 x0[KS], x1[KS];
    auto fill = [&](double2 (&x)[KS], int q, int pstep) {
      const int li = max(li_lo, min(li_hi, q + pstep * step));
      const double2 *xp = xs + li;
#pragma unroll
      for (int s = 0; s < KS; ++s) x[s] = xp[4 * s];
    };
    int qc = qof(qcd, qci) + lane_li;
    fill(x0, qc, pc);

    int left = t1 - t0;
    auto tile = [&](const double2 (&xc)[KS], double2 (&xn)[KS]) {
      int wrap;
      asm("s_lshr_b32 %0, %1, 31" : "=s"(wrap) : "s"(pend - 8 - pc));
      const int gnext = g + wrap;
      int pnext = pc + 4, pend_next = pend;
      if (wrap != 0 && left > 1) {
        if constexpr (KS & 1) asm volatile("v_cvt_i32_f64 %0, %1" : "=v"(qc) : "v"(qnd));
        else asm volatile("v_mov_b32 %0, %1" : "=v"(qc) : "v"(qni));
        qc += lane_li;
        if (gnext == wr.b1 || gnext == wr.b2) {
          p0 = __builtin_amdgcn_readfirstlane(walk_p0(fw, gnext));
          pend_next = __builtin_amdgcn_readfirstlane(p0 + 4 * walk_ncs(fw, fb.K, kb, ke, gnext));
        }
        pnext = p0;
      }
      fill(xn, qc, left > 1 ? pnext : pc);
      double accA = 0.0, accB = 0.0;
#pragma unroll
      for (int s = 0; s < KS; ++s) {
        accA = __builtin_amdgcn_mfma_f64_4x4x4f64(cc[s], xc[s].x, accA, 0, 0, 0);
        accB = __builtin_amdgcn_mfma_f64_4x4x4f64(cc[s], xc[s].y, accB, 0, 0, 0);
      }
      (void)x0;
      const int ib = lane_ib + 16 * g + pc * pl;
      if constexpr (OGEN) {
        if ((unsigned)ib < (unsigned)cnt && 16 * g + rloc < pl) {
          const long long A = oabs0 + ib;
          E *const p = (A >= io.out_abs0 && A < io.out_end) ? oext + (A - io.out_abs0) * io.nch : oring + (A & io.out_ring_mask) * io.nch;
          if (io.out_unaligned) {
            p[0] = Fr::out(accA);
            p[1] = Fr::out(accB);
          } else
            *reinterpret_cast<E2 *>(p) = E2{Fr::out(accA), Fr::out(accB)};
        }
      } else if constexpr (OUT64) {
        const bool ok = (unsigned)ib < (unsigned)cnt && 16 * g + rloc < pl;
        const unsigned off = ok ? ((o64 + (unsigned)ib) & m64) * 8u : 0xffffffffu;
        const rsmp_v2u da = {(unsigned)__double2loint(accA), (unsigned)__double2hiint(accA)};
        const rsmp_v2u db = {(unsigned)__double2loint(accB), (unsigned)__double2hiint(accB)};
        __builtin_amdgcn_raw_buffer_store_b64(da, orsrcA, (int)off, 0, 0);
        __builtin_amdgcn_raw_buffer_store_b64(db, orsrcB, (int)off, 0, 0);
      } else {
        unsigned off = (unsigned)(lane_off0 + (16 * g + pc * pl) * frame_bytes);
        if (g == ngrp - 1 && (pl & 15)) {
          off = lane_dead_last ? 0xffffffffu : off;
          asm volatile("" : "+v"(off));
        }
        if constexpr (sizeof(E) == 8) {
          const rsmp_v4u d = {(unsigned)__double2loint(accA), (unsigned)__double2hiint(accA), (unsigned)__double2loint(accB),
                              (unsigned)__double2hiint(accB)};
          __builtin_amdgcn_raw_buffer_store_b128(d, orsrc, (int)off, 0, 0);
        } else if constexpr (sizeof(E) == 2) {
          __builtin_amdgcn_raw_buffer_store_b32(pcm_pack16(accA, accB), orsrc, (int)off, 0, 0);
        } else if constexpr (std::is_same<E, int>::value) {
          const rsmp_v2u d = {(unsigned)pcm_out32(accA), (unsigned)pcm_out32(accB)};
          __builtin_amdgcn_raw_buffer_store_b64(d, orsrc, (int)off, 0, 0);
        } else {
          const rsmp_v2u d = {__float_as_uint((float)accA), __float_as_uint((float)accB)};
          __builtin_amdgcn_raw_buffer_store_b64(d, orsrc, (int)off, 0, 0);
        }
      }
      if (wrap != 0 && left > 1) {
#pragma unroll
        for (int s = 0; s < KS; ++s) asm volatile("v_mov_b64 %0, %1" : "=v"(cc[s]) : "v"(cn[s]));
        __builtin_amdgcn_sched_barrier(0);
        load_tile(min(gnext + 1, ngrp - 1), cn, qnd, qni);
      }
      g = gnext;
      pc = pnext;
      pend = pend_next;
      --left;
    };
    while (true) {
      tile(x0, x1);
      if (left == 0) break;
      tile(x1, x0);
      if (left == 0) break;
    }
  };

  const bool run = fb.cnt > 0;
  if constexpr (SPLIT && TWO) {
    if (run) poly_round(0, fw.ka, smp, -kPad, min(V, kSplitRaEnd) + kPad - 4 * KS);
    __syncthreads();
    {
      double2 *l2 = reinterpret_cast<double2 *>(lds);
#pragma unroll
      for (int s = kSplitSB0; s < 16; ++s) {
        const int n = 2 * (tid + s * T);
        if (n < V) {
          l2[n - kSplitRbStart] = make_double2(z0[s].x, z0[s].y);
          l2[n + 1 - kSplitRbStart] = make_double2(v[s].x, v[s].y);
        }
      }
      if (tid < kPad && V > kSplitRbStart) l2[V - kSplitRbStart + tid] = make_double2(0.0, 0.0);
    }
    __syncthreads();
    if (tail_in_b) store_tail(reinterpret_cast<const double2 *>(lds), kSplitRbStart);
    if (run && fw.ka < fb.K) poly_round(fw.ka, fb.K, reinterpret_cast<const double2 *>(lds) - kSplitRbStart, kSplitRbStart, V + kPad - 4 * KS);
    return;
  } else if constexpr (SPLIT) {
    if (run) poly_round(0, fb.K, smp, -kPad, V + kPad - 4 * KS);
    return;
  }
  if (run) poly_round(0, fw.ka, smp, -kPad, min(V, kSA * T) + kPad - 4 * KS);
  RSMP_STAMP(6)
  __syncthreads();
  {
    double2 *l2 = reinterpret_cast<double2 *>(lds);
#pragma unroll
    for (int s = kSB0; s < 16; ++s) {
      const int n = tid + s * T;
      if (n < V) l2[n - kSB0 * T] = make_double2(v[s].x, v[s].y);
    }
    if (tid < kPad && V > kSB0 * T) l2[V - kSB0 * T + tid] = make_double2(0.0, 0.0);
  }
  __syncthreads();
  if (tail_in_b) store_tail(reinterpret_cast<const double2 *>(lds), kSB0 * T);
  if (run && fw.ka < fb.K) poly_round(fw.ka, fb.K, reinterpret_cast<const double2 *>(lds) - kSB0 * T, kSB0 * T, V + kPad - 4 * KS);
  RSMP_STAMP(5)
#ifdef RSMP_STAMPS_BUILD
  if (stamping && tid == 0) atomicAdd(a.stamps + 7, 1ull);
#endif
#undef RSMP_STAMP
}

template <int LOG2P, int KS, bool OUT64>
__global__ __launch_bounds__(256, kFusedWaves) void fused_fast_kernel(FusedArgs a, FastIo io)
{
  fused_fast_body<LOG2P, KS, OUT64, false, false>(a, io);
}
template <int KS, int OMODE>
__global__ __launch_bounds__(256, 2) void fused_split_kernel(FusedArgs a, FastIo io)
{
  fused_fast_body<12, KS, OMODE == 1, true, OMODE == 2>(a, io);
}
template <int KS, int OMODE>
__global__ __launch_bounds__(256, 2) void fused_split2_kernel(FusedArgs a, FastIo io)
{
  fused_fast_body<12, KS, OMODE == 1, true, OMODE == 2, true>(a, io);
}

template <int LOG2P, int KS, bool OUT64>
__global__ __launch_bounds__(256, kFusedWaves) void fused_fast_dio_kernel(FusedArgs a, FastIo io)
{
  fused_fast_body<LOG2P, KS, OUT64, false, false, false, double>(a, io);
}
template <int KS, int OMODE>
__global__ __launch_bounds__(256, 2) void fused_split_dio_kernel(FusedArgs a, FastIo io)
{
  fused_fast_body<12, KS, OMODE == 1, true, OMODE == 2, false, double>(a, io);
}
template <int KS, int OMODE>
__global__ __launch_bounds__(256, 2) void fused_split2_dio_kernel(FusedArgs a, FastIo io)
{
  fused_fast_body<12, KS, OMODE == 1, true, OMODE == 2, true, double>(a, io);
}

#define RSMP_PCM_KERNELS(tag, E)                                                                                          \
  template <int LOG2P, int KS, bool OUT64>                                                                                \
  __global__ __launch_bounds__(256, kFusedWaves) void fused_fast_##tag##_kernel(FusedArgs a, FastIo io)                  \
  {                                                                                                                       \
    fused_fast_body<LOG2P, KS, OUT64, false, false, false, E>(a, io);                                                     \
  }                                                                                                                       \
  template <int KS, int OMODE> __global__ __launch_bounds__(256, 2) void fused_split_##tag##_kernel(FusedArgs a, FastIo io) \
  {                                                                                                                       \
    fused_fast_body<12, KS, OMODE == 1, true, OMODE == 2, false, E>(a, io);                                               \
  }                                                                                                                       \
  template <int KS, int OMODE> __global__ __launch_bounds__(256, 2) void fused_split2_##tag##_kernel(FusedArgs a, FastIo io) \
  {                                                                                                                       \
    fused_fast_body<12, KS, OMODE == 1, true, OMODE == 2, true, E>(a, io);                                                \
  }
RSMP_PCM_KERNELS(s16, short)
RSMP_PCM_KERNELS(s32, int)
#undef RSMP_PCM_KERNELS

typedef void (*FastKernel)(FusedArgs, FastIo);

template <int LOG2P, int KS, bool OUT64> static hipError_t launch_fast_t(const FusedArgs &a, const FastIo &io, hipStream_t st)
{
  constexpr int N = 4096;
  size_t lds_bytes = 8 * size_t(fft_lds_doubles_halves(12));
  if (LOG2P < 12) lds_bytes = std::max(lds_bytes, 8 * size_t(std::max(fft_lds_doubles(LOG2P), fft8_lds_doubles(LOG2P))));
  lds_bytes = std::max(lds_bytes, size_t(kPad + kSA * (N / 16) + kPad) * 16);
  static DynLdsOnce attr[4];
  static const FastKernel fns[4] = {&fused_fast_kernel<LOG2P, KS, OUT64>, &fused_fast_dio_kernel<LOG2P, KS, OUT64>,
                                    &fused_fast_s16_kernel<LOG2P, KS, OUT64>, &fused_fast_s32_kernel<LOG2P, KS, OUT64>};
  if (io.dio < 0 || io.dio > 3) return hipErrorInvalidValue;
  if (hipError_t e = attr[io.dio].set(reinterpret_cast<const void *>(fns[io.dio]), int(lds_bytes)); e != hipSuccess) return e;
  FusedArgs b = a;
  b.d.hp = io.nch >= 4 ? io.nch / 2 : 0;
  dim3 grid(item_grid(a.d.nblocks, a.d.C / 2, b.d.hp)), block(N / 16);
  hipLaunchKernelGGL(fns[io.dio], grid, block, lds_bytes, st, b, io);
  return hipGetLastError();
}

template <int KS, int OMODE, bool TWO> static hipError_t launch_split_t(const FusedArgs &a, const FastIo &io, hipStream_t st)
{
  const size_t lds_max = std::max(size_t(8) * fft_lds_doubles_halves(12), size_t(kPad + (TWO ? kSplitRaEnd : kSplitVsMax) + kPad) * 16);
  const size_t lds_bytes = TWO ? lds_max : std::max(size_t(8) * fft_lds_doubles_halves(12), size_t(kPad + a.d.Vs + kPad) * 16);
  static DynLdsOnce attr[4];
  static const FastKernel fns[4] = {
      TWO ? &fused_split2_kernel<KS, OMODE> : &fused_split_kernel<KS, OMODE>, TWO ? &fused_split2_dio_kernel<KS, OMODE> : &fused_split_dio_kernel<KS, OMODE>,
      TWO ? &fused_split2_s16_kernel<KS, OMODE> : &fused_split_s16_kernel<KS, OMODE>, TWO ? &fused_split2_s32_kernel<KS, OMODE> : &fused_split_s32_kernel<KS, OMODE>};
  if (io.dio < 0 || io.dio > 3) return hipErrorInvalidValue;
  if (hipError_t e = attr[io.dio].set(reinterpret_cast<const void *>(fns[io.dio]), int(lds_max)); e != hipSuccess) return e;
  FusedArgs b = a;
  b.d.hp = io.nch >= 4 ? io.nch / 2 : 0;
  dim3 grid(item_grid(a.d.nblocks, a.d.C / 2, b.d.hp)), block(256);
  hipLaunchKernelGGL(fns[io.dio], grid, block, lds_bytes, st, b, io);
  return hipGetLastError();
}

bool fused_split_two_supported(int V, int taps, int ksteps, int qb_spread)
{
  return !knobs().no_split2 && !(V & 1) && V == 8192 - (taps - 1) && V > kSplitVsMax && V - kSplitRbStart + kPad <= kSplitRaEnd + kPad &&
         qb_spread + 4 * ksteps + 4 <= kSplitRaEnd - kSplitRbStart + kPad && ksteps >= 7 && ksteps <= 9;
}

bool fused_split_supported(int log2n, int L, int ksteps)
{
  return !knobs().no_fast && !knobs().no_split && L == 2 && log2n >= 13 && log2n <= 15 && ksteps >= 7 && ksteps <= 9;
}

hipError_t launch_fused_split(int omode, const FusedArgs &a, const FastIo &io, hipStream_t st, const char **kname)
{
  if (a.d.two) {
    if (a.d.nsub != 1 || a.d.Vs != a.d.V || a.d.Pref != 4096 || a.d.V <= kSplitVsMax || a.d.V > 8192 || (a.d.V & 1)) return hipErrorInvalidValue;
  } else if (a.d.Vs > kSplitVsMax) return hipErrorInvalidValue;
  if (a.d.nsub < 1 || a.d.Vs < 64 || (a.d.Vs & 1) || (a.d.V & 1) || a.d.nblocks % a.d.nsub || omode < 0 || omode > 2 ||
      (omode == 1 ? !io.out64 : omode == 2 ? !io.out_ring : !io.out) ||
      (a.d.Pref != 4096 && a.d.Pref != 8192 && a.d.Pref != 16384) || a.d.nsub * a.d.Vs < a.d.V || (a.d.nsub - 1) * a.d.Vs >= a.d.V || (io.nch & 1))
    return hipErrorInvalidValue;
  for (int i = 0; i < a.d.nsub; ++i) {
    const SubBlock sb = sub_block(i, a.d.V, a.d.Vs, a.d.Pref);
    const int ov = 2 * a.d.Pref - a.d.V;
    if (sb.win < 0 || sb.shift < 0 || sb.shift + sb.len / 2 + (ov + 1) / 2 > 4096 || (sb.len & 1) || sb.win + 4096 > a.d.Pref) return hipErrorInvalidValue;
  }
#define RSMP_IO_NAME(fmt, head, tail) \
  ((fmt) == 1 ? head "_dio_" tail : (fmt) == 2 ? head "_s16_" tail : (fmt) == 3 ? head "_s32_" tail : head "_" tail)
#define RSMP_SPLIT_CASE(ks, om)                                                        \
  if (a.KS == ks && omode == om && !a.d.two) {                                         \
    if (kname) *kname = RSMP_IO_NAME(io.dio, "rsmp::fused_split", "kernel<" #ks ", " #om ">");  \
    return launch_split_t<ks, om, false>(a, io, st);                                   \
  }                                                                                    \
  if (a.KS == ks && omode == om && a.d.two) {                                          \
    if (kname) *kname = RSMP_IO_NAME(io.dio, "rsmp::fused_split2", "kernel<" #ks ", " #om ">"); \
    return launch_split_t<ks, om, true>(a, io, st);                                    \
  }
  RSMP_SPLIT_CASE(7, 0) RSMP_SPLIT_CASE(7, 1) RSMP_SPLIT_CASE(7, 2) RSMP_SPLIT_CASE(8, 0) RSMP_SPLIT_CASE(8, 1) RSMP_SPLIT_CASE(8, 2)
  RSMP_SPLIT_CASE(9, 0) RSMP_SPLIT_CASE(9, 1) RSMP_SPLIT_CASE(9, 2)
#undef RSMP_SPLIT_CASE
  return hipErrorInvalidValue;
}

size_t fused_walk_enumerate(const FusedPrepArgs &p, int k, long long *head, int *slots, size_t cap)
{
  const FusedBlock fb = fused_block_info(p, k);
  const int pl = p.polyL, step = p.step, ngrp = (pl + 15) >> 4;
  const FusedWalk fw = fused_walk(fb, ngrp);
  const FusedWalk uni = {0, ngrp, fb.KA};
  const long long h[13] = {fb.i_lo, fb.cnt, fb.K, fb.KA, fb.walk < 0, fw.g_lo, fw.g_hi, fw.ka,
                           fb.cnt > 0 ? fused_walk_tiles(fw, fb.K, ngrp) : 0, fb.cnt > 0 ? fused_walk_tiles(uni, fb.K, ngrp) : 0,
                           fb.irel_lo, fb.base_li, ngrp};
  for (int i = 0; i < 13; ++i) head[i] = h[i];
  size_t n = 0;
  if (fb.cnt <= 0) return 0;
  for (int round = 0; round < 2; ++round) {
    const int kb = round ? fw.ka : 0, ke = round ? fb.K : fw.ka;
    if (ke <= kb) continue;
    const WalkRound wr = walk_round(fw, fb.K, kb, ke, ngrp);
    const int cnt = walk_round_cnt(fb, fw, ke, pl);
    for (int wave = 0; wave < 4; ++wave) {
      const int t0 = (wr.nt * wave) >> 2, t1 = (wr.nt * (wave + 1)) >> 2;
      if (t0 >= t1) continue;
      int g, c;
      walk_seek(wr, t0, g, c);
      int pc = 4 * c + walk_p0(fw, g), pend = walk_p0(fw, g) + 4 * walk_ncs(fw, fb.K, kb, ke, g);
      for (int left = t1 - t0; left > 0; --left) {
        for (int lane = 0; lane < 64; ++lane) {
          const int hi = lane >> 4, bq = (lane >> 2) & 3, jq = lane & 3, rloc = 4 * bq + hi;
          const long long a0 = p.at0 + (long long)(16 * g + 4 * bq) * step;
          const int li = walk_lane_li(fb, kb, hi, jq, step) + int(a0 / pl) + pc * step;
          const int ib = walk_lane_ib(fb, kb, jq, rloc, pl) + 16 * g + pc * pl;
          if (n < cap) {
            int *o = slots + 7 * n;
            o[0] = round, o[1] = g, o[2] = (pc - walk_p0(fw, g)) >> 2, o[3] = lane, o[4] = ib;
            o[5] = ib >= 0 && ib < cnt && 16 * g + rloc < pl;
            o[6] = li;
          }
          ++n;
        }
        if (pc + 4 == pend) {
          ++g;
          pc = walk_p0(fw, g);
          pend = pc + 4 * walk_ncs(fw, fb.K, kb, ke, g);
        } else
          pc += 4;
      }
    }
  }
  return n;
}

bool fused_fast_supported(int log2n, int log2p, int ksteps)
{
  return !knobs().no_fast && log2n == 12 && (log2p == 11 || log2p == 12) && (ksteps == 7 || ksteps == 8);
}

#define RSMP_FAST_CASE(p, ks)                                                                        \
  if (log2p == p && a.KS == ks) {                                                                    \
    if (kname) *kname = io.out64 ? RSMP_IO_NAME(io.dio, "rsmp::fused_fast", "kernel<" #p ", " #ks ", true>") \
                                 : RSMP_IO_NAME(io.dio, "rsmp::fused_fast", "kernel<" #p ", " #ks ", false>"); \
    return io.out64 ? launch_fast_t<p, ks, true>(a, io, st) : launch_fast_t<p, ks, false>(a, io, st); \
  }

hipError_t launch_fused_fast(int log2p, const FusedArgs &a, const FastIo &io, hipStream_t st, const char **kname)
{
  RSMP_FAST_CASE(11, 7) RSMP_FAST_CASE(12, 7) RSMP_FAST_CASE(11, 8) RSMP_FAST_CASE(12, 8)
  return hipErrorInvalidValue;
}

}
```

### foo_dsp_resampler_amd/csrc/kernels.hpp

```cpp
#pragma once
#include <hip/hip_runtime.h>
#include <atomic>
#include <cstdint>

#include "knobs.hpp"

namespace rsmp {

struct DynLdsOnce {
  std::atomic<unsigned long long> mask{0};
  hipError_t set(const void *fn, int bytes)
  {
    int dev = 0;
    hipError_t e = hipGetDevice(&dev);
    if (e != hipSuccess) return e;
    if (dev < 64 && ((mask.load(std::memory_order_acquire) >> dev) & 1ull)) return hipSuccess;
    e = hipFuncSetAttribute(fn, hipFuncAttributeMaxDynamicSharedMemorySize, bytes);
    if (e == hipSuccess && dev < 64) mask.fetch_or(1ull << dev, std::memory_order_release);
    return e;
  }
};

enum { kRingF64 = 0, kFramesF32 = 1, kFramesF64 = 2, kFramesS16 = 3, kFramesS32 = 4 };
__host__ __device__ constexpr int frame_elem_bytes(int kind) { return kind == kFramesF64 ? 8 : kind == kFramesS16 ? 2 : 4; }

__host__ __device__ __forceinline__ double pcm_in(short s) { return (double)s * 0x1p-15; }
__host__ __device__ __forceinline__ double pcm_in(int s) { return (double)s * 0x1p-31; }
__host__ __device__ __forceinline__ short pcm_out16(double y)
{
  return (short)(int)fmin(fmax(rint(y * 32768.0), -32768.0), 32767.0);
}
__host__ __device__ __forceinline__ int pcm_out32(double y)
{
  return (int)fmin(fmax(rint(y * 2147483648.0), -2147483648.0), 2147483647.0);
}
__host__ __device__ __forceinline__ unsigned pcm_pack16(double a, double b)
{
  return (unsigned)(unsigned short)pcm_out16(a) | ((unsigned)(unsigned short)pcm_out16(b) << 16);
}
__host__ __device__ __forceinline__ double pcm_lo16(unsigned w) { return pcm_in((short)(w & 0xffffu)); }
__host__ __device__ __forceinline__ double pcm_hi16(unsigned w) { return pcm_in((short)(w >> 16)); }
struct FrameView {
  void *ring;
  long long ring_mask;
  long long ring_stream_stride;
  void *ext;
  long long ext_begin, ext_end;
  long long ext_stream_stride;
  int nch;
};

struct RingView {
  double *ring;
  long long mask;
  long long chan_stride;
};

struct AnyView {
  int kind;
  FrameView f;
  RingView d;
};

struct DftArgs {
  const double2 *G;
  const double2 *Gr;
  const double2 *tw_fwd;
  const double2 *tw_inv;
  const double2 *tw_fwd8;
  const double2 *tw_inv8;
  long long B0;
  long long out_offset;
  int nblocks;
  int C;
  int L;
  int c0;
  int V;
  int Vout;
  int q;
  int M;
  int nchs;
  int npairs;
  unsigned pps_magic;
  int hp;
  long long in_limit;
  long long clip_lo, clip_hi;
  int nsub, Vs;
  int two;
  int Pref;
  long long Bref0;
};

struct SubBlock { int off, len, win, shift; };
__host__ __device__ inline SubBlock sub_block(int i, int V, int Vs, int Pref)
{
  SubBlock s;
  s.off = i * Vs;
  s.len = V - s.off < Vs ? V - s.off : Vs;
  s.win = (s.off >> 1) < Pref - 4096 ? (s.off >> 1) : Pref - 4096;
  s.shift = (s.off >> 1) - s.win;
  return s;
}

__host__ __device__ inline int pair_count(int C, int nchs) { return nchs > 0 ? (C / nchs) * ((nchs + 1) >> 1) : (C + 1) >> 1; }

__host__ __device__ inline unsigned pair_magic(int C, int nchs)
{
  const unsigned long long pps = (unsigned long long)(((nchs > 0 ? nchs : C) + 1) >> 1);
  return pps <= 1 ? 0u : (unsigned)(((1ull << 32) + pps - 1) / pps);
}

struct BigDftArgs {
  DftArgs d;
  const double2 *twN;
  double2 *w1, *w2;
  int log2n, log2mp, log2md;
  int fdomain_in;
  int item0;
};
bool big_dft_supported(int log2n, int log2p, int log2nd);
hipError_t launch_dft_big(const AnyView &in, const AnyView &out, BigDftArgs a, int ws_items, hipStream_t st);

struct FusedBlock {
  long long i_lo;
  int cnt;
  int irel_lo;
  int base_li;
  int K;
  int KA;
  int walk;
  long long seam_i0;
  int seam_q0, seam_ph0;
};
constexpr int kFusedSA = 12, kFusedSB0 = 10, kFusedWaves = 3;

struct FusedWalk { int g_lo, g_hi, ka; };
__host__ __device__ inline FusedWalk fused_walk(const FusedBlock &fb, int ngrp)
{
  if (fb.walk >= 0) return FusedWalk{0, ngrp, fb.KA};
  return FusedWalk{fb.walk & 1023, (fb.walk >> 10) & 1023, (fb.walk >> 20) & 2047};
}
__host__ __device__ inline int walk_p0(const FusedWalk &w, int g) { return g < w.g_lo ? 1 : 0; }
__host__ __device__ inline int walk_ncs(const FusedWalk &w, int K, int kb, int ke, int g)
{
  const int p0 = walk_p0(w, g), pend = g >= w.g_hi ? K - 1 : K;
  const int e = ke + p0 < pend ? ke + p0 : pend, n = (e - kb - p0 + 3) >> 2;
  return n > 0 ? n : 1;
}
struct WalkRound { int b1, b2, n0, n1, n2, T1, T2, nt; };
__host__ __device__ inline WalkRound walk_round(const FusedWalk &w, int K, int kb, int ke, int ngrp)
{
  WalkRound r;
  const int lo = w.g_lo < ngrp ? w.g_lo : ngrp, hi = w.g_hi < ngrp ? w.g_hi : ngrp;
  r.b1 = lo < hi ? lo : hi;
  r.b2 = lo < hi ? hi : lo;
  r.n0 = walk_ncs(w, K, kb, ke, 0);
  r.n1 = walk_ncs(w, K, kb, ke, r.b1);
  r.n2 = walk_ncs(w, K, kb, ke, r.b2);
  r.T1 = r.b1 * r.n0;
  r.T2 = r.T1 + (r.b2 - r.b1) * r.n1;
  r.nt = r.T2 + (ngrp - r.b2) * r.n2;
  return r;
}
__host__ __device__ inline void walk_seek(const WalkRound &r, int t, int &g, int &c)
{
  int gb = 0, tb = 0, n = r.n0;
  if (t >= r.T2) {
    gb = r.b2, tb = r.T2, n = r.n2;
  } else if (t >= r.T1) {
    gb = r.b1, tb = r.T1, n = r.n1;
  }
  const int dg = (t - tb) / n;
  g = gb + dg;
  c = t - tb - dg * n;
}
__host__ __device__ inline int walk_lane_li(const FusedBlock &fb, int kb, int hi, int jq, int step) { return fb.base_li + hi + (kb + jq) * step; }
__host__ __device__ inline int walk_lane_ib(const FusedBlock &fb, int kb, int jq, int rloc, int pl) { return (kb + jq) * pl + rloc - fb.irel_lo; }
__host__ __device__ inline int walk_round_cnt(const FusedBlock &fb, const FusedWalk &w, int ke, int pl)
{
  const int irel_hi = fb.irel_lo + fb.cnt, e = (ke + (w.g_lo > 0 ? 1 : 0)) * pl;
  return (irel_hi < e ? irel_hi : e) - fb.irel_lo;
}
__host__ __device__ inline int fused_walk_tiles(const FusedWalk &w, int K, int ngrp)
{
  return (w.ka > 0 ? walk_round(w, K, 0, w.ka, ngrp).nt : 0) + (w.ka < K ? walk_round(w, K, w.ka, K, ngrp).nt : 0);
}

struct FusedPrepArgs {
  long long b_offset, B0, at0;
  int V, polyL, step, n, nblocks;
  int two_round, KS, qb_max;
  int ra_end, rb_start;
  int qb_min;
  long long clip_lo, clip_hi;
  int nsub, Vs;
};
__host__ __device__ inline FusedBlock fused_block_info(const FusedPrepArgs &p, int k)
{
  long long b0 = p.b_offset + (p.B0 + k) * (long long)p.V;
  int V = p.V;
  if (p.nsub > 0) {
    const int kr = k / p.nsub, i = k - kr * p.nsub;
    b0 = p.b_offset + (p.B0 + kr) * (long long)p.V + (long long)i * p.Vs;
    V = p.V - i * p.Vs < p.Vs ? p.V - i * p.Vs : p.Vs;
  }
  const long long nlo = b0 * p.polyL - p.at0, nhi = (b0 + V - p.n + 1) * p.polyL - p.at0;
  long long ilo = nlo <= 0 ? 0 : (nlo + p.step - 1) / p.step, ihi = nhi <= 0 ? 0 : (nhi + p.step - 1) / p.step;
  if (ilo < p.clip_lo) ilo = p.clip_lo;
  if (ihi > p.clip_hi) ihi = p.clip_hi;
  FusedBlock fb;
  fb.i_lo = ilo;
  fb.cnt = ihi > ilo ? int(ihi - ilo) : 0;
  const long long kk_lo = ilo / p.polyL;
  fb.irel_lo = int(ilo - kk_lo * p.polyL);
  fb.base_li = int(kk_lo * p.step - b0);
  fb.K = fb.cnt > 0 ? int((ihi - 1) / p.polyL - kk_lo) + 1 : 0;
  fb.KA = fb.K;
  int fit = fb.K;
  {
    const long long ns = (b0 - (p.n - 1)) * p.polyL - p.at0;
    const long long s0 = ns <= 0 ? 0 : (ns + p.step - 1) / p.step;
    const long long a0 = p.at0 + s0 * p.step, q0 = a0 / p.polyL;
    fb.seam_i0 = s0;
    fb.seam_q0 = int(q0 - (b0 - (p.n - 1)));
    fb.seam_ph0 = int(a0 - q0 * p.polyL);
  }
  const int ra_end = p.ra_end > 0 ? p.ra_end : kFusedSA * 256, rb_start = p.ra_end > 0 ? p.rb_start : kFusedSB0 * 256;
  if (p.two_round && V > ra_end) {
    const int a_hi = ra_end + 32 - 4 * p.KS - 3, num = a_hi - fb.base_li - p.qb_max;
    const int ka = num < 0 ? 0 : num / p.step + 1;
    fb.KA = ka < fb.K ? ka : fb.K;
    const int k4 = fb.KA & ~3;
    if (fb.KA < fb.K && k4 > 0 && fb.base_li + p.qb_min + k4 * p.step >= rb_start) fb.KA = k4;
    fit = ka;
  }
  fb.walk = 0;
  const int ngrp = (p.polyL + 15) >> 4;
  if (fb.cnt > 0 && ngrp <= 1023 && fb.K <= 2047) {
    FusedWalk w;
    w.g_lo = fb.irel_lo >> 4;
    w.g_hi = (fb.irel_lo + fb.cnt - 1 - (fb.K - 1) * p.polyL + 16) >> 4;
    w.ka = fb.K;
    const int p1 = w.g_lo > 0 ? 1 : 0;
    const int maxlen = w.g_lo < w.g_hi ? fb.K : fb.K - 1;
    int best = -1, best_ka = 0;
    if (fit >= fb.K) {
      best = fused_walk_tiles(w, fb.K, ngrp);
      best_ka = fb.K;
    } else {
      for (int a4 = 4; a4 + p1 <= fit; a4 += 4) {
        const bool all = a4 >= maxlen;
        if (!all && fb.base_li + p.qb_min + a4 * p.step < rb_start) continue;
        w.ka = all ? fb.K : a4;
        const int t = fused_walk_tiles(w, fb.K, ngrp);
        if (best < 0 || t < best) {
          best = t;
          best_ka = w.ka;
        }
        if (all) break;
      }
    }
    const FusedWalk u = {0, ngrp, fb.KA};
    if (best >= 0 && best <= fused_walk_tiles(u, fb.K, ngrp))
      fb.walk = int(0x80000000u | unsigned(w.g_lo) | unsigned(w.g_hi) << 10 | unsigned(best_ka) << 20);
  }
  return fb;
}
constexpr int kFusedMaxBlocks = 1024;

struct FusedArgs {
  DftArgs d;
  const double *tab;
  const double *cft;
  double *seam;
  long long at0;
  long long b_offset;
  long long out_offset2;
  int seam_mask;
  int n, polyL, step;
  int span;
  int NG, KC;
  int kper;
  const double *cfm;
  int NGRP, KS;
  int reserved = 0;
  unsigned long long *stamps;
  const FusedBlock *blk;
  const int *qtab;
  const double2 *cfm2;
};

struct FastIo {
  const void *in;
  const void *in_ring;
  long long in_ring_mask, in_ring_stream_stride;
  void *out;
  long long in_abs0, out_abs0;
  long long in_stream_stride, out_stream_stride;
  int nch;
  int in_unaligned;
  void *out_ring;
  long long out_ring_mask, out_ring_stream_stride, out_end;
  int out_unaligned;
  double *out64;
  long long out64_mask, out64_chan_stride;
  int dio;
};
bool fused_fast_supported(int log2n, int log2p, int ksteps);
hipError_t launch_fused_fast(int log2p, const FusedArgs &a, const FastIo &io, hipStream_t st, const char **kname = nullptr);
constexpr int kSplitVsMax = 5056;
constexpr int kSplitSA = 9, kSplitSB0 = 8, kSplitRaEnd = 2 * kSplitSA * 256, kSplitRbStart = 2 * kSplitSB0 * 256;
bool fused_split_supported(int log2n, int L, int ksteps);
hipError_t launch_fused_split(int omode, const FusedArgs &a, const FastIo &io, hipStream_t st, const char **kname = nullptr);
bool fused_split_two_supported(int V, int taps, int ksteps, int qb_spread);

struct PolyArgs {
  const double *tab;
  long long rd;
  long long at;
  long long step;
  long long out_abs;
  long long count;
  int C, n, L, phase_bits, tile, win;
  int tab_lds;
  int coop;
  int shared_rows;
};

struct HalfArgs {
  long long rd, out_abs, count;
  int C, ncoef, pre;
  double coef[13];
};

hipError_t launch_dft(int log2n, int log2p, int log2nd, const AnyView &in, const AnyView &out, const DftArgs &a, hipStream_t st,
                      const char **kname = nullptr);
hipError_t launch_poly(int order, const AnyView &in, const AnyView &out, const PolyArgs &a, hipStream_t st, const char **kname = nullptr);
hipError_t launch_half(const AnyView &in, const AnyView &out, const HalfArgs &a, hipStream_t st, const char **kname = nullptr);
bool dft_shape_supported(int log2n, int log2p, int log2nd);
bool dftx_supported(int log2n, int log2p, int log2nd);
hipError_t launch_dftx(int log2n, const AnyView &in, const AnyView &out, const DftArgs &a, hipStream_t st, const char **kname = nullptr);
hipError_t launch_fused(int log2n, int log2p, const AnyView &in, const AnyView &out, const FusedArgs &a, hipStream_t st,
                        const char **kname = nullptr);
hipError_t launch_seam(const AnyView &out, const FusedArgs &a, hipStream_t st);
bool fused_shape_supported(int log2n, int log2p, int n, int span, int max_seam_outputs);
bool fused_mfma_supported(int log2n, int log2p, int ksteps);
hipError_t launch_fused_prep(const FusedPrepArgs &p, FusedBlock *out, hipStream_t st);
size_t fused_walk_enumerate(const FusedPrepArgs &p, int k, long long *head, int *slots, size_t cap);

struct PolyMfArgs {
  const double *cfm;
  const int *qtab;
  const FusedBlock *blk;
  long long B0;
  long long at0;
  long long out_offset;
  long long in_limit;
  int nblocks, C, Vt, n, polyL, step, NGRP;
  int nchs, npairs;
  unsigned pps_magic;
};
bool polymf_supported(int ksteps);
hipError_t launch_polymf(int ksteps, const AnyView &in, const AnyView &out, const PolyMfArgs &a, hipStream_t st,
                         const char **kname = nullptr);
hipError_t launch_copy(const AnyView &in, const AnyView &out, long long a0, long long a1, int C, hipStream_t st);

}
```

### foo_dsp_resampler_amd/ratelib.py

```python
import ctypes as C
import json
import os

import numpy as np

HERE = os.path.dirname(os.path.abspath(__file__))
RR_BEST, RR_NORM = 0, 1

EXPECTED_SYMBOLS = [
    "init_ratelib", "close_ratelib", "RR_open", "RR_flow", "RR_push", "RR_pull", "RR_drain", "RR_close", "RR_strerror",
    "RRX_open_batch", "RRX_open_batch_on", "RRX_device", "RRX_push_device", "RRX_pull_device", "RRX_flow_device", "RRX_push_strided", "RRX_pull_strided",
    "RRX_set_stream", "RRX_sync", "RRX_profile", "RRX_profile_read", "RRX_profile_report", "RRX_debug_fail_alloc",
    "RRX_debug_tile_walk",
    "RRX_open_batch_fmt", "RRX_format", "RRX_push_double", "RRX_pull_double", "RRX_flow_double", "RRX_push_device_double",
    "RRX_pull_device_double", "RRX_flow_device_double",
    "RRX_push_samples", "RRX_pull_samples", "RRX_flow_samples", "RRX_push_device_samples", "RRX_pull_device_samples",
    "RRX_flow_device_samples",
    "RRX_lpc_extrapolate_device", "RRX_edge_geometry",
    "RRX_finish_device", "RRX_debug_finish_host",
    "RRX_isamp_max", "RRX_available", "RRX_channels", "RRX_streams",
    "RRX_describe_plan", "RRX_describe_dispatch", "RRX_plan_table",
]
RRX_FMT_FLOAT, RRX_FMT_DOUBLE = 0, 1
RRX_FMT_S16, RRX_FMT_S32 = 16, 32
RRX_FMT_S24_3 = 24
_FMT_DTYPE = {RRX_FMT_FLOAT: np.dtype(np.float32), RRX_FMT_DOUBLE: np.dtype(np.float64), RRX_FMT_S16: np.dtype(np.int16),
              RRX_FMT_S32: np.dtype(np.int32)}
_DTYPE_FMT = {d: f for f, d in _FMT_DTYPE.items()}


class RRConfig(C.Structure):
    _fields_ = [("in_rate", C.c_size_t), ("out_rate", C.c_size_t), ("phase", C.c_double),
                ("bandwidth", C.c_double), ("allow_aliasing", C.c_int), ("quality", C.c_int)]


class WalkGeom(C.Structure):
    _fields_ = [("at0", C.c_longlong), ("b_offset", C.c_longlong), ("B0", C.c_longlong)] + [
        (k, C.c_int) for k in ("V", "polyL", "step", "n", "KS", "qb_min", "qb_max", "two_round", "ra_end", "rb_start", "nsub", "Vs")]


class RRError(RuntimeError):
    def __init__(self, code, what):
        self.code = code
        super().__init__("%s failed: %d (%s)" % (what, code, lib().RR_strerror(code).decode()))


def lib_path():
    return os.environ.get("RATELIB_AMD_SO") or os.path.join(HERE, "libratelib_amd.so")


_lib = None
_ALLOC_CB = C.CFUNCTYPE(None)


alloc_handler_calls = 0


def _alloc_failed():
    global alloc_handler_calls
    alloc_handler_calls += 1


_alloc_cb = _ALLOC_CB(_alloc_failed)
_inited = False


def _share_hip_runtime_with_torch():
    try:
        import importlib.util
        spec = importlib.util.find_spec("torch")
        if spec is None or not spec.origin:
            return None
        p = os.path.join(os.path.dirname(spec.origin), "lib", "libamdhip64.so")
        if os.path.exists(p):
            return C.CDLL(p, mode=C.RTLD_GLOBAL)
    except Exception:
        pass
    return None


_hip_rt = None


def lib():
    global _lib, _hip_rt
    if _lib is None:
        p = lib_path()
        if not os.path.exists(p):
            raise RuntimeError("libratelib_amd.so is not built; run `python -m foo_dsp_resampler_amd.build`")
        _hip_rt = _share_hip_runtime_with_torch()
        L = C.CDLL(p)
        P = C.POINTER
        vp, sz = C.c_void_p, C.c_size_t
        L.init_ratelib.argtypes = [_ALLOC_CB]
        L.RR_open.argtypes = [P(RRConfig), C.c_int, P(vp)]
        L.RRX_open_batch.argtypes = [P(RRConfig), C.c_int, C.c_int, P(vp)]
        L.RRX_open_batch_on.argtypes = [P(RRConfig), C.c_int, C.c_int, C.c_int, P(vp)]
        L.RRX_device.argtypes = [vp]
        L.RRX_open_batch_fmt.argtypes = [P(RRConfig), C.c_int, C.c_int, C.c_int, C.c_int, P(vp)]
        L.RRX_format.argtypes = [vp]
        L.RRX_push_double.argtypes = [vp, vp, sz, sz]
        L.RRX_pull_double.argtypes = [vp, vp, sz, sz, P(sz)]
        L.RRX_flow_double.argtypes = [vp, vp, sz, vp, sz, sz, sz, P(sz), P(sz)]
        L.RRX_push_device_double.argtypes = [vp, vp, sz, sz]
        L.RRX_pull_device_double.argtypes = [vp, vp, sz, sz, P(sz)]
        L.RRX_flow_device_double.argtypes = [vp, vp, sz, vp, sz, sz, sz, P(sz), P(sz)]
        L.RRX_push_samples.argtypes = [vp, C.c_int, vp, sz, sz]
        L.RRX_pull_samples.argtypes = [vp, C.c_int, vp, sz, sz, P(sz)]
        L.RRX_flow_samples.argtypes = [vp, C.c_int, vp, sz, vp, sz, sz, sz, P(sz), P(sz)]
        L.RRX_push_device_samples.argtypes = [vp, C.c_int, vp, sz, sz]
        L.RRX_pull_device_samples.argtypes = [vp, C.c_int, vp, sz, sz, P(sz)]
        L.RRX_flow_device_samples.argtypes = [vp, C.c_int, vp, sz, vp, sz, sz, sz, P(sz), P(sz)]
        L.RR_push.argtypes = [vp, vp, sz]
        L.RR_pull.argtypes = [vp, vp, sz, P(sz)]
        L.RR_flow.argtypes = [vp, vp, vp, sz, sz, P(sz), P(sz)]
        L.RR_drain.argtypes = [vp]
        L.RR_close.argtypes = [P(vp)]
        L.RR_close.restype = None
        L.RR_strerror.argtypes = [C.c_int]
        L.RR_strerror.restype = C.c_char_p
        L.RRX_push_device.argtypes = [vp, vp, sz, sz]
        L.RRX_pull_device.argtypes = [vp, vp, sz, sz, P(sz)]
        L.RRX_flow_device.argtypes = [vp, vp, sz, vp, sz, sz, sz, P(sz), P(sz)]
        L.RRX_push_strided.argtypes = [vp, vp, sz, sz]
        L.RRX_pull_strided.argtypes = [vp, vp, sz, sz, P(sz)]
        L.RRX_set_stream.argtypes = [vp, vp]
        L.RRX_sync.argtypes = [vp]
        L.RRX_profile.argtypes = [vp, C.c_int]
        L.RRX_profile_read.argtypes = [vp, P(C.c_double), P(C.c_longlong), P(C.c_double), P(C.c_longlong)]
        L.RRX_profile_report.argtypes = [vp, C.c_char_p, sz]
        L.RRX_debug_fail_alloc.argtypes = [C.c_int]
        L.RRX_debug_fail_alloc.restype = None
        if hasattr(L, "RRX_debug_tile_walk"):
            L.RRX_debug_tile_walk.argtypes = [P(WalkGeom), C.c_int, P(C.c_longlong), vp, sz]
            L.RRX_debug_tile_walk.restype = C.c_longlong
        for n in ("RRX_isamp_max", "RRX_available"):
            getattr(L, n).argtypes = [vp]
            getattr(L, n).restype = sz
        L.RRX_channels.argtypes = [vp]
        L.RRX_streams.argtypes = [vp]
        L.RRX_describe_plan.argtypes = [P(RRConfig), C.c_char_p, sz]
        L.RRX_describe_dispatch.argtypes = [P(RRConfig), C.c_int, C.c_char_p, sz]
        L.RRX_plan_table.argtypes = [P(RRConfig), C.c_int, vp, sz, P(sz)]
        if hasattr(L, "RRX_lpc_extrapolate_device"):
            L.RRX_lpc_extrapolate_device.argtypes = [C.c_int, vp, vp, sz, C.c_int, sz, C.c_int, C.c_int, sz, sz]
            L.RRX_edge_geometry.argtypes = [sz, sz, P(sz), P(sz), P(sz), P(sz)]
        if hasattr(L, "RRX_finish_device"):
            u64 = C.c_ulonglong
            host = [C.c_int, vp, sz, C.c_int, vp, sz, C.c_int, sz, C.c_int, vp, C.c_int, u64, u64, vp, vp]
            L.RRX_finish_device.argtypes = [C.c_int, vp] + host
            L.RRX_debug_finish_host.argtypes = host
        _lib = L
    return _lib


def available_symbols():
    L = lib()
    return [s for s in EXPECTED_SYMBOLS if hasattr(L, s)]


def _config(in_rate, out_rate, phase=50.0, bandwidth=95.0, allow_aliasing=0, quality=RR_BEST):
    return RRConfig(int(in_rate), int(out_rate), float(phase), float(bandwidth), int(allow_aliasing), int(quality))


def describe_plan(in_rate, out_rate, **kw):
    cfg = _config(in_rate, out_rate, **kw)
    buf = C.create_string_buffer(1 << 16)
    n = lib().RRX_describe_plan(C.byref(cfg), buf, len(buf))
    if n < 0:
        raise RRError(-n, "RRX_describe_plan")
    return json.loads(buf.value.decode())


def describe_dispatch(in_rate, out_rate, nch, **kw):
    cfg = _config(in_rate, out_rate, **kw)
    buf = C.create_string_buffer(1 << 14)
    n = lib().RRX_describe_dispatch(C.byref(cfg), int(nch), buf, len(buf))
    if n < 0:
        raise RRError(-n, "RRX_describe_dispatch")
    return json.loads(buf.value.decode())


def plan_table(which, in_rate, out_rate, **kw):
    cfg = _config(in_rate, out_rate, **kw)
    n = C.c_size_t(0)
    rc = lib().RRX_plan_table(C.byref(cfg), which, None, 0, C.byref(n))
    if rc:
        raise RRError(rc, "RRX_plan_table")
    out = np.empty(n.value, dtype=np.float64)
    if n.value:
        lib().RRX_plan_table(C.byref(cfg), which, out.ctypes.data, n.value, C.byref(n))
    return out


def edge_geometry(in_rate, out_rate):
    v = [C.c_size_t(0) for _ in range(4)]
    _check(lib().RRX_edge_geometry(int(in_rate), int(out_rate), *[C.byref(x) for x in v]), "RRX_edge_geometry")
    return tuple(x.value for x in v)


def lpc_extrapolate_device(t, first, data_len, extra_bkwd, extra_fwd, order=32, stream=None):
    shape = tuple(t.shape)
    if len(shape) not in (2, 3):
        raise ValueError("expected a [frames, nch] or [nstreams, frames, nch] tensor, got shape %r" % (shape,))
    if not str(t.dtype).endswith("float32"):
        raise TypeError("%s buffer: the LPC extrapolator works on float32 frames only" % (t.dtype,))
    if not t.is_contiguous():
        raise ValueError("the tensor must be contiguous")
    nstreams, frames, nch = (1,) + shape if len(shape) == 2 else shape
    first, data_len, extra_bkwd, extra_fwd = int(first), int(data_len), int(extra_bkwd), int(extra_fwd)
    if min(first, data_len, extra_bkwd, extra_fwd) < 0 or first < extra_bkwd or first + data_len + extra_fwd > frames:
        raise ValueError("frames [%d, %d) do not lie inside the tensor's %d frames"
                         % (first - extra_bkwd, first + data_len + extra_fwd, frames))
    _ensure_init()
    index = getattr(getattr(t, "device", None), "index", None)
    ptr = getattr(stream, "cuda_stream", stream) or 0
    _check(lib().RRX_lpc_extrapolate_device(-1 if index is None else int(index), C.c_void_p(ptr),
                                            C.c_void_p(t.data_ptr() + first * nch * 4), frames, nstreams, data_len, nch, int(order),
                                            extra_bkwd, extra_fwd), "RRX_lpc_extrapolate_device")


def finish_device(x, dst_format, gain=None, dither=False, seed=0, first_frame=0, out=None, peak=None, clipped=None, stream=None):
    import torch
    shape = tuple(x.shape)
    if len(shape) not in (2, 3):
        raise ValueError("expected a [frames, nch] or [nstreams, frames, nch] tensor, got shape %r" % (shape,))
    dt = str(x.dtype)
    if not (dt.endswith("float32") or dt.endswith("float64")):
        raise TypeError("%s buffer: the output stage reads float32 or float64 frames" % (x.dtype,))
    if not x.is_contiguous():
        raise ValueError("the tensor must be contiguous")
    if dst_format not in (None, RRX_FMT_S16, RRX_FMT_S24_3, RRX_FMT_S32):
        raise ValueError("unknown dst_format %r (RRX_FMT_S16, RRX_FMT_S24_3, RRX_FMT_S32 or None)" % (dst_format,))
    nstreams, frames, nch = (1,) + shape if len(shape) == 2 else shape
    seed, first_frame = int(seed), int(first_frame)
    if not (0 <= seed < 1 << 64 and 0 <= first_frame and first_frame + frames < 1 << 64):
        raise ValueError("seed and first_frame + frames must fit 64 unsigned bits")
    if not getattr(x, "is_cuda", False):
        raise TypeError("the output stage works on device tensors: the frames must be in HBM")
    dev = x.device
    if gain is not None and not hasattr(gain, "data_ptr"):
        gain = torch.full((nstreams,), float(gain), dtype=torch.float64, device=dev)
    if gain is not None:
        if gain.dtype != torch.float64 or tuple(gain.shape) != (nstreams,) or gain.device != dev or not gain.is_contiguous():
            raise TypeError("gain must be a float, or a contiguous float64 tensor [%d] on %s" % (nstreams, dev))
    if dst_format is None:
        if out is not None:
            raise ValueError("dst_format=None measures only: there is nothing to write into `out`")
    else:
        odt, last = {RRX_FMT_S16: (torch.int16, nch), RRX_FMT_S32: (torch.int32, nch), RRX_FMT_S24_3: (torch.uint8, nch * 3)}[dst_format]
        oshape = shape[:-1] + (last,)
        if out is None:
            out = torch.empty(oshape, dtype=odt, device=dev)
        elif out.dtype != odt or tuple(out.shape) != oshape or out.device != dev or not out.is_contiguous():
            raise TypeError("out must be a contiguous %s tensor %r on %s" % (odt, oshape, dev))
    stats = []
    for t, sdt, name in ((peak, torch.float64, "peak"), (clipped, torch.int64, "clipped")):
        if t is None:
            t = torch.zeros((nstreams, nch), dtype=sdt, device=dev)
        elif t.dtype != sdt or tuple(t.shape) != (nstreams, nch) or t.device != dev or not t.is_contiguous():
            raise TypeError("%s must be a contiguous %s tensor [%d, %d] on %s" % (name, sdt, nstreams, nch, dev))
        stats.append(t)
    peak, clipped = stats
    _ensure_init()
    ptr = getattr(stream, "cuda_stream", stream) or 0
    _check(lib().RRX_finish_device(-1 if dev.index is None else int(dev.index), C.c_void_p(ptr),
                                   RRX_FMT_DOUBLE if dt.endswith("float64") else RRX_FMT_FLOAT, C.c_void_p(x.data_ptr()), frames,
                                   dst_format or 0, C.c_void_p(out.data_ptr()) if out is not None else None, frames, nstreams, frames, nch,
                                   C.c_void_p(gain.data_ptr()) if gain is not None else None, 1 if dither else 0, seed, first_frame,
                                   C.c_void_p(peak.data_ptr()), C.c_void_p(clipped.data_ptr())), "RRX_finish_device")
    return out, peak, clipped


def _ensure_init():
    global _inited
    if not _inited:
        if lib().init_ratelib(_alloc_cb) != 0:
            raise RuntimeError("init_ratelib failed: no usable HIP device (the engine has no CPU path)")
        _inited = True


def _check(rc, what):
    if rc:
        raise RRError(rc, what)


class Resampler:

# ... 300 lines not shown
```

### include/ratelib_amd.h

```cpp
#ifndef RATELIB_AMD_H
#define RATELIB_AMD_H

#include "ratelib.h"

#ifdef __cplusplus
extern "C" {
#endif

int RRX_open_batch(const RR_config *config, int nchannels, int nstreams, RR_handle **const handle);

int RRX_open_batch_on(const RR_config *config, int nchannels, int nstreams, int device, RR_handle **const handle);
int RRX_device(const RR_handle *h);

int RRX_push_device(RR_handle *h, const fb_sample_t *d_ibuf, size_t in_stride, size_t isamp);
int RRX_pull_device(RR_handle *h, fb_sample_t *d_obuf, size_t out_stride, size_t osamp, size_t *ogen);
int RRX_flow_device(RR_handle *h, const fb_sample_t *d_ibuf, size_t in_stride, fb_sample_t *d_obuf, size_t out_stride,
                    size_t isamp, size_t osamp, size_t *iused, size_t *ogen);

int RRX_push_strided(RR_handle *h, const fb_sample_t *ibuf, size_t in_stride, size_t isamp);
int RRX_pull_strided(RR_handle *h, fb_sample_t *obuf, size_t out_stride, size_t osamp, size_t *ogen);

#define RRX_STREAM_OWN ((void *)(~(size_t)0))
int RRX_set_stream(RR_handle *h, void *hip_stream);
int RRX_sync(RR_handle *h);

int RRX_profile(RR_handle *h, int enable);
int RRX_profile_read(RR_handle *h, double *hot_ms, long long *hot_launches, double *other_ms, long long *other_launches);
int RRX_profile_report(RR_handle *h, char *buf, size_t cap);

void RRX_debug_fail_alloc(int nth);

typedef struct RRX_walk_geom {
  long long at0, b_offset, B0;
  int V, polyL, step, n, KS, qb_min, qb_max, two_round, ra_end, rb_start, nsub, Vs;
} RRX_walk_geom;
long long RRX_debug_tile_walk(const RRX_walk_geom *geom, int k, long long *head, int *slots, size_t cap);

#define RRX_FMT_FLOAT  0
#define RRX_FMT_DOUBLE 1
int RRX_open_batch_fmt(const RR_config *config, int nchannels, int nstreams, int device, int format, RR_handle **const handle);
int RRX_format(const RR_handle *h);

int RRX_push_double(RR_handle *h, const double *ibuf, size_t in_stride, size_t isamp);
int RRX_pull_double(RR_handle *h, double *obuf, size_t out_stride, size_t osamp, size_t *ogen);
int RRX_flow_double(RR_handle *h, const double *ibuf, size_t in_stride, double *obuf, size_t out_stride,
                    size_t isamp, size_t osamp, size_t *iused, size_t *ogen);
int RRX_push_device_double(RR_handle *h, const double *d_ibuf, size_t in_stride, size_t isamp);
int RRX_pull_device_double(RR_handle *h, double *d_obuf, size_t out_stride, size_t osamp, size_t *ogen);
int RRX_flow_device_double(RR_handle *h, const double *d_ibuf, size_t in_stride, double *d_obuf,
                           size_t out_stride, size_t isamp, size_t osamp, size_t *iused, size_t *ogen);

#define RRX_FMT_S16 16
#define RRX_FMT_S32 32

int RRX_push_samples(RR_handle *h, int format, const void *ibuf, size_t in_stride, size_t isamp);
int RRX_pull_samples(RR_handle *h, int format, void *obuf, size_t out_stride, size_t osamp, size_t *ogen);
int RRX_flow_samples(RR_handle *h, int format, const void *ibuf, size_t in_stride, void *obuf, size_t out_stride,
                     size_t isamp, size_t osamp, size_t *iused, size_t *ogen);
int RRX_push_device_samples(RR_handle *h, int format, const void *d_ibuf, size_t in_stride, size_t isamp);
int RRX_pull_device_samples(RR_handle *h, int format, void *d_obuf, size_t out_stride, size_t osamp, size_t *ogen);
int RRX_flow_device_samples(RR_handle *h, int format, const void *d_ibuf, size_t in_stride, void *d_obuf, size_t out_stride,
                            size_t isamp, size_t osamp, size_t *iused, size_t *ogen);

int RRX_lpc_extrapolate_device(int device, void *hip_stream, fb_sample_t *d_data, size_t stream_stride, int nstreams,
                               size_t data_len, int nch, int lpc_order, size_t extra_bkwd, size_t extra_fwd);

#define RRX_FMT_S24_3 24
int RRX_finish_device(int device, void *hip_stream, int src_format, const void *d_src, size_t src_stride,
                      int dst_format, void *d_dst, size_t dst_stride, int nstreams, size_t frames, int nch,
                      const double *d_gain, int dither, unsigned long long seed, unsigned long long first_frame,
                      double *d_peak, unsigned long long *d_clipped);
int RRX_debug_finish_host(int src_format, const void *src, size_t src_stride, int dst_format, void *dst, size_t dst_stride,
                          int nstreams, size_t frames, int nch, const double *gain, int dither, unsigned long long seed,
                          unsigned long long first_frame, double *peak, unsigned long long *clipped);

int RRX_edge_geometry(size_t in_rate, size_t out_rate, size_t *n_add, size_t *n_drop, size_t *prime_len, size_t *inbuf);

size_t RRX_isamp_max(const RR_handle *h);
size_t RRX_available(const RR_handle *h);
int RRX_channels(const RR_handle *h);
int RRX_streams(const RR_handle *h);

int RRX_describe_plan(const RR_config *config, char *buf, size_t cap);

int RRX_describe_dispatch(const RR_config *config, int nchannels, char *buf, size_t cap);

int RRX_plan_table(const RR_config *config, int which, double *out, size_t cap, size_t *count);

#ifdef __cplusplus
}
#endif

#endif
```

Before: 124,900 Msamples/s.

## Precompute per-block walk start state in prep kernel and prefetch coefficient tiles early

The prep kernel now also computes, per block and per round, the walk start state (group, phase, end, boundary groups) and stores it in a device table. The fused fast kernel reads it through scalar constant-address loads instead of recomputing the walk seek and per-group divisions in every workgroup. It also issues the coefficient tile loads earlier, overlapping them with the FFT and seam phases. This trades extra register pressure and a larger prep kernel for less scalar arithmetic and latency in the polyphase stage.

```diff
diff --git a/foo_dsp_resampler_amd/csrc/capi.cpp b/foo_dsp_resampler_amd/csrc/capi.cpp
--- a/foo_dsp_resampler_amd/csrc/capi.cpp
+++ b/foo_dsp_resampler_amd/csrc/capi.cpp
@@ -343,11 +343,10 @@
 
 void RRX_debug_fail_alloc(int nth) { rsmp::Engine::fail_alloc_after(nth); }
 
-long long RRX_debug_tile_walk(const RRX_walk_geom *g, int k, long long *head, int *slots, size_t cap)
-{
-  if (!rsmp::knobs().test_hooks || !g || !head || (cap && !slots) || k < 0) return -1;
-  if (g->polyL < 1 || g->step < 1 || g->V < 1 || g->n < 1 || g->KS < 1 || g->nsub < 0 || (g->nsub > 0 && g->Vs < 1)) return -1;
-  rsmp::FusedPrepArgs pa;
+static bool walk_geom_args(const RRX_walk_geom *g, int k, rsmp::FusedPrepArgs &pa)
+{
+  if (!rsmp::knobs().test_hooks || !g || k < 0) return false;
+  if (g->polyL < 1 || g->step < 1 || g->V < 1 || g->n < 1 || g->KS < 1 || g->nsub < 0 || (g->nsub > 0 && g->Vs < 1)) return false;
   pa.b_offset = g->b_offset;
   pa.B0 = g->B0;
   pa.at0 = g->at0;
@@ -366,7 +365,23 @@
   pa.clip_hi = 0x7fffffffffffffffLL;
   pa.nsub = g->nsub;
   pa.Vs = g->Vs;
+  return true;
+}
+
+long long RRX_debug_tile_walk(const RRX_walk_geom *g, int k, long long *head, int *slots, size_t cap)
+{
+  rsmp::FusedPrepArgs pa;
+  if (!head || (cap && !slots) || !walk_geom_args(g, k, pa)) return -1;
   return (long long)rsmp::fused_walk_enumerate(pa, k, head, slots, cap);
+}
+
+int RRX_debug_walk_start(const RRX_walk_geom *g, int k, RRX_walk_start *out)
+{
+  rsmp::FusedPrepArgs pa;
+  if (!out || !walk_geom_args(g, k, pa)) return -1;
+  static_assert(sizeof(RRX_walk_start) == 56 * sizeof(int), "RRX_walk_start mirrors rsmp::WalkStart");
+  rsmp::fused_walk_start_host(pa, k, reinterpret_cast<int *>(out));
+  return 0;
 }
 
 int RRX_lpc_extrapolate_device(int device, void *hip_stream, fb_sample_t *d_data, size_t stream_stride, int nstreams, size_t data_len,
diff --git a/foo_dsp_resampler_amd/csrc/engine.cpp b/foo_dsp_resampler_amd/csrc/engine.cpp
--- a/foo_dsp_resampler_amd/csrc/engine.cpp
+++ b/foo_dsp_resampler_amd/csrc/engine.cpp
@@ -422,6 +422,7 @@
   while (fu.blk_cap < 8 * split_nsub) fu.blk_cap *= 2;
   fu.slots = 2 * fu.blk_cap;
   ALLOC_TRY(&fu.blk_dev, size_t(2 * fu.blk_cap) * sizeof(FusedBlock));
+  ALLOC_TRY(&fu.wst_dev, size_t(2 * fu.blk_cap) * sizeof(WalkStart));
   const size_t bytes = size_t(C_ + 1) * fu.slots * 2 * 32 * sizeof(double);
   ALLOC_TRY(&fu.seam, bytes);
   HIP_TRY(hipMemset(fu.seam, 0, bytes));
@@ -656,6 +657,7 @@
     if (f.cfm2) (void)hipFree(f.cfm2);
     if (f.Gs) (void)hipFree(f.Gs);
     if (f.blk_dev) (void)hipFree(f.blk_dev);
+    if (f.wst_dev) (void)hipFree(f.wst_dev);
   }
   for (BigDft &b : big_) {
     if (b.twN) (void)hipFree(b.twN);
@@ -1001,8 +1003,10 @@
   const bool seam_on_side = more_slabs && !(profiling_ || !dst_frames || no_side_);
   if (seam_launches_ >= 2) HIP_TRY(hipStreamWaitEvent(stream_, ev_seam_[seam_launches_ & 1], 0));
   FusedBlock *const blk_half = fu.blk_dev + size_t(seam_launches_ & 1) * fu.blk_cap;
-  { const int pp = prof_begin(false, "rsmp::fused_prep_kernel"); HIP_TRY(launch_fused_prep(pa, blk_half, stream_)); prof_end(pp); }
+  WalkStart *const wst_half = fu.wst_dev + size_t(seam_launches_ & 1) * fu.blk_cap;
+  { const int pp = prof_begin(false, "rsmp::fused_prep_kernel"); HIP_TRY(launch_fused_prep(pa, blk_half, stream_, wst_half)); prof_end(pp); }
   fa.blk = blk_half;
+  fa.wst = wst_half;
   const long long endnum = (b.wr[i] - sp.n + 1) * sp.L - fa.at0;
   if (wro - out_offset + count != (endnum <= 0 ? 0 : (endnum + step - 1) / step)) return kInternal;
   const bool in_frames = i - 1 == 0;
@@ -1096,6 +1100,7 @@
     fr.d.B0 = fa.d.B0 + b0;
     fr.d.nblocks = b1 - b0;
     fr.blk = fa.blk + b0;
+    fr.wst = fa.wst + b0;
     const int pi = prof_begin(true);
     const char *kn = nullptr;
     if (fast) HIP_TRY(launch_fused_fast(pend_log2p, fr, io, stream_, &kn));
diff --git a/foo_dsp_resampler_amd/csrc/engine.hpp b/foo_dsp_resampler_amd/csrc/engine.hpp
--- a/foo_dsp_resampler_amd/csrc/engine.hpp
+++ b/foo_dsp_resampler_amd/csrc/engine.hpp
@@ -142,7 +142,7 @@
   std::vector<BigDft> big_;
   struct Fuse { bool on = false; int span = 0, NG = 0, KC = 0, kper = 0; double *seam = nullptr; double *cft = nullptr; int slots = 0;
                 double *cfm = nullptr; int NGRP = 0, KS = 0, qb_max = 0, qb_min = 0; int *qtab = nullptr; double2 *cfm2 = nullptr;
-                FusedBlock *blk_dev = nullptr; int blk_cap = 0;
+                FusedBlock *blk_dev = nullptr; int blk_cap = 0; WalkStart *wst_dev = nullptr;
                 int nsub = 0, Vs = 0; double2 *Gs = nullptr; };
   std::vector<Fuse> fuse_;
   struct PolyMf { double *cfm = nullptr; int *qtab = nullptr; FusedBlock *blk = nullptr; int KS = 0, NGRP = 0, Vt = 0, blk_cap = 0; };
diff --git a/foo_dsp_resampler_amd/csrc/fused.hip b/foo_dsp_resampler_amd/csrc/fused.hip
--- a/foo_dsp_resampler_amd/csrc/fused.hip
+++ b/foo_dsp_resampler_amd/csrc/fused.hip
@@ -511,15 +511,18 @@
   }
 }
 
-__global__ __launch_bounds__(256) void fused_prep_kernel(FusedPrepArgs p, FusedBlock *out)
-{
-  const int k = blockIdx.x * 256 + threadIdx.x;
-  if (k < p.nblocks) out[k] = fused_block_info(p, k);
-}
-
-hipError_t launch_fused_prep(const FusedPrepArgs &p, FusedBlock *out, hipStream_t st)
-{
-  hipLaunchKernelGGL(fused_prep_kernel, dim3((p.nblocks + 255) / 256), dim3(256), 0, st, p, out);
+__global__ __launch_bounds__(256) void fused_prep_kernel(FusedPrepArgs p, FusedBlock *out, WalkStart *wst)
+{
+  const int t = blockIdx.x * 256 + threadIdx.x, k = t >> 1, round = t & 1;
+  if (k >= p.nblocks || (round && !wst)) return;
+  const FusedBlock fb = fused_block_info(p, k);
+  if (!round) out[k] = fb;
+  if (wst) fused_walk_start_round(fb, (p.polyL + 15) >> 4, p.polyL, round, wst[k].r[round]);
+}
+
+hipError_t launch_fused_prep(const FusedPrepArgs &p, FusedBlock *out, hipStream_t st, WalkStart *wst)
+{
+  hipLaunchKernelGGL(fused_prep_kernel, dim3((2 * p.nblocks + 255) / 256), dim3(256), 0, st, p, out, wst);
   return hipGetLastError();
 }
 
diff --git a/foo_dsp_resampler_amd/csrc/fused_fast.hip b/foo_dsp_resampler_amd/csrc/fused_fast.hip
--- a/foo_dsp_resampler_amd/csrc/fused_fast.hip
+++ b/foo_dsp_resampler_amd/csrc/fused_fast.hip
@@ -6,6 +6,7 @@
 #include <atomic>
 #include <cstdlib>
 #include <cstdio>
+#include <cstring>
 #include <type_traits>
 
 namespace rsmp {
@@ -68,6 +69,25 @@
   }
   const int V = SPLIT ? sb.len : a.d.V;
   const bool fwd_active = tid < TF;
+  constexpr bool TAB_AT_START = LOG2P == LOG2N - 1 && !SPLIT, EARLY_TILES = !SPLIT;
+  constexpr bool TILES_A_FIRST = TAB_AT_START && EARLY_TILES && KS <= 7;
+  typedef const int __attribute__((address_space(4))) *TabPtr;
+  const int lane = tid & 63, wave = __builtin_amdgcn_readfirstlane(tid >> 6);
+  struct { long long i_lo; int cnt, irel_lo, base_li; } fb;
+  struct RoundStart { int kb, cnt, b1, b2, p01, p02, pe1, pe2, n, g, pc, pend; };
+  RoundStart rsA, rsB;
+  auto fetch_table = [&] {
+    const TabPtr tb = (TabPtr)(const void *)(a.blk + bl), ts = (TabPtr)(const void *)(a.wst + bl);
+    fb.i_lo = (long long)(((unsigned long long)(unsigned)tb[1] << 32) | (unsigned)tb[0]);
+    fb.cnt = tb[2], fb.irel_lo = tb[3], fb.base_li = tb[4];
+    auto round_start = [&](int r) {
+      const TabPtr q = ts + r * (int)(sizeof(WalkStartRound) / 4), w = q + 12 + 4 * wave;
+      return RoundStart{q[0], q[2], q[3], q[4], q[6], q[7], q[9], q[10], w[0], w[1], w[2], w[3]};
+    };
+    rsA = round_start(0);
+    rsB = round_start(1);
+  };
+  if constexpr (TAB_AT_START) fetch_table();
   const double2 *__restrict__ Gp = a.d.G;
   double2 *smp = reinterpret_cast<double2 *>(lds) + kPad;
   const int nm1 = a.n - 1;
@@ -194,6 +214,35 @@
   if constexpr (!SPLIT) fft_regs<LOG2N, +1, 2, kPfInv>(v, tid, true, a.d.tw_inv, lds);
   RSMP_STAMP(3)
 
+  const int hi = lane >> 4, bq = (lane >> 2) & 3, jq = lane & 3;
+  const int rloc = 4 * bq + hi;
+  const int ngrp = a.NGRP;
+  const double2 *const cfm_lane = a.cfm2 + lane;
+  const int *const qtab_lane = a.qtab + bq;
+
+  double cc[KS], cn[KS];
+  double qcd = 0.0, qnd = 0.0;
+  int qci = 0, qni = 0;
+  auto load_tile = [&](int gg, double (&c_)[KS], double &qd_, int &qi_) {
+    constexpr int KSP = (KS + 1) / 2;
+    const double2 *cp = cfm_lane + gg * (KSP * 64);
+#pragma unroll
+    for (int s2 = 0; s2 < KSP; ++s2) {
+      const double2 d = cp[s2 * 64];
+      c_[2 * s2] = d.x;
+      if (2 * s2 + 1 < KS) c_[2 * s2 + 1] = d.y;
+      else qd_ = d.y;
+    }
+    if (!(KS & 1)) qi_ = qtab_lane[gg * 4];
+  };
+  auto request_tiles = [&](const RoundStart &rs) {
+    load_tile(rs.g, cc, qcd, qci);
+    load_tile(min(rs.g + 1, ngrp - 1), cn, qnd, qni);
+  };
+  if constexpr (!TAB_AT_START) fetch_table();
+  if constexpr (TILES_A_FIRST) request_tiles(rsA);
+
+
   const int ca = 2 * pair, cb = ca + 1;
   {
     const int slot = (int)(B & a.seam_mask);
@@ -246,6 +295,7 @@
     }
     }
   }
+  if constexpr (EARLY_TILES && !TILES_A_FIRST) request_tiles(rsA);
   __syncthreads();
   if constexpr (SPLIT) {
     if (tid < nm1) {
@@ -268,9 +318,6 @@
   if (!tail_in_b) store_tail(smp, 0);
   RSMP_STAMP(4)
 
-  const FusedBlock fb = a.blk[bl];
-  const int lane = tid & 63, wave = __builtin_amdgcn_readfirstlane(tid >> 6);
-  const int hi = lane >> 4, bq = (lane >> 2) & 3, jq = lane & 3;
   const int pl = a.polyL, step = a.step;
   const int frame_bytes = io.nch * (int)sizeof(E);
   char *const obytes = (OUT64 || OGEN) ? nullptr
@@ -286,49 +333,20 @@
     orsrcA = __builtin_amdgcn_make_buffer_rsrc(ra, 0, (int)((io.out64_mask + 1) * 8), 0x00020000);
     orsrcB = __builtin_amdgcn_make_buffer_rsrc(ra + io.out64_chan_stride, 0, (int)((io.out64_mask + 1) * 8), 0x00020000);
   }
-  const int rloc = 4 * bq + hi;
-  const int ngrp = a.NGRP;
-  const double2 *const cfm_lane = a.cfm2 + lane;
-  const int *const qtab_lane = a.qtab + bq;
-
-  const FusedWalk fw = fused_walk(fb, ngrp);
-  auto poly_round = [&](int kb, int ke, const double2 *xs, int li_lo, int li_hi) {
-    if (ke <= kb) return;
-    const WalkRound wr = walk_round(fw, fb.K, kb, ke, ngrp);
-    const int t0 = (wr.nt * wave) >> 2, t1 = (wr.nt * (wave + 1)) >> 2;
-    if (t0 >= t1) return;
-    int g, pc;
-    walk_seek(wr, t0, g, pc);
-    g = __builtin_amdgcn_readfirstlane(g);
-    int p0 = __builtin_amdgcn_readfirstlane(walk_p0(fw, g));
-    pc = __builtin_amdgcn_readfirstlane(4 * pc + p0);
-    int pend = __builtin_amdgcn_readfirstlane(p0 + 4 * walk_ncs(fw, fb.K, kb, ke, g));
-    const int lane_li = walk_lane_li(fb, kb, hi, jq, step);
-    const int lane_ib = walk_lane_ib(fb, kb, jq, rloc, pl);
-    const int cnt = walk_round_cnt(fb, fw, ke, pl);
+  auto poly_round = [&](const RoundStart &rs, const double2 *xs, int li_lo, int li_hi) {
+    if (rs.n == 0) return;
+    if constexpr (!EARLY_TILES) request_tiles(rs);
+    const int kb = rs.kb;
+    int g = rs.g, pc = rs.pc, pend = rs.pend;
+    int p0 = pc & 3;
+    const int lane_li = walk_lane_li(fb.base_li, kb, hi, jq, step);
+    const int lane_ib = walk_lane_ib(fb.irel_lo, kb, jq, rloc, pl);
+    const int cnt = rs.cnt;
     const __amdgpu_buffer_rsrc_t orsrc =
         __builtin_amdgcn_make_buffer_rsrc(obytes, 0, (!OUT64 && !OGEN && cnt > 0) ? (cnt - 1) * frame_bytes + 2 * (int)sizeof(E) : 0, 0x00020000);
     const int lane_off0 = __mul24(lane_ib, frame_bytes);
     const bool lane_dead_last = 16 * (ngrp - 1) + rloc >= pl;
-
-    double cc[KS], cn[KS];
-    double qcd = 0.0, qnd = 0.0;
-    int qci = 0, qni = 0;
-    auto load_tile = [&](int gg, double (&c_)[KS], double &qd_, int &qi_) {
-      constexpr int KSP = (KS + 1) / 2;
-      const double2 *cp = cfm_lane + gg * (KSP * 64);
-#pragma unroll
-      for (int s2 = 0; s2 < KSP; ++s2) {
-        const double2 d = cp[s2 * 64];
-        c_[2 * s2] = d.x;
-        if (2 * s2 + 1 < KS) c_[2 * s2 + 1] = d.y;
-        else qd_ = d.y;
-      }
-      if (!(KS & 1)) qi_ = qtab_lane[gg * 4];
-    };
     auto qof = [&](double qd_, int qi_) { return (KS & 1) ? (int)qd_ : qi_; };
-    load_tile(g, cc, qcd, qci);
-    load_tile(min(g + 1, ngrp - 1), cn, qnd, qni);
 
     double2 x0[KS], x1[KS];
     auto fill = [&](double2 (&x)[KS], int q, int pstep) {
@@ -340,7 +358,7 @@
     int qc = qof(qcd, qci) + lane_li;
     fill(x0, qc, pc);
 
-    int left = t1 - t0;
+    int left = rs.n;
     auto tile = [&](const double2 (&xc)[KS], double2 (&xn)[KS]) {
       int wrap;
       asm("s_lshr_b32 %0, %1, 31" : "=s"(wrap) : "s"(pend - 8 - pc));
@@ -350,10 +368,8 @@
         if constexpr (KS & 1) asm volatile("v_cvt_i32_f64 %0, %1" : "=v"(qc) : "v"(qnd));
         else asm volatile("v_mov_b32 %0, %1" : "=v"(qc) : "v"(qni));
         qc += lane_li;
-        if (gnext == wr.b1 || gnext == wr.b2) {
-          p0 = __builtin_amdgcn_readfirstlane(walk_p0(fw, gnext));
-          pend_next = __builtin_amdgcn_readfirstlane(p0 + 4 * walk_ncs(fw, fb.K, kb, ke, gnext));
-        }
+        if (gnext == rs.b2) p0 = rs.p02, pend_next = rs.pe2;
+        else if (gnext == rs.b1) p0 = rs.p01, pend_next = rs.pe1;
         pnext = p0;
       }
       fill(xn, qc, left > 1 ? pnext : pc);
@@ -423,7 +439,8 @@
 
   const bool run = fb.cnt > 0;
   if constexpr (SPLIT && TWO) {
-    if (run) poly_round(0, fw.ka, smp, -kPad, min(V, kSplitRaEnd) + kPad - 4 * KS);
+    if (run) poly_round(rsA, smp, -kPad, min(V, kSplitRaEnd) + kPad - 4 * KS);
+    if constexpr (EARLY_TILES) request_tiles(rsB);
     __syncthreads();
     {
       double2 *l2 = reinterpret_cast<double2 *>(lds);
@@ -439,13 +456,14 @@
     }
     __syncthreads();
     if (tail_in_b) store_tail(reinterpret_cast<const double2 *>(lds), kSplitRbStart);
-    if (run && fw.ka < fb.K) poly_round(fw.ka, fb.K, reinterpret_cast<const double2 *>(lds) - kSplitRbStart, kSplitRbStart, V + kPad - 4 * KS);
+    if (run) poly_round(rsB, reinterpret_cast<const double2 *>(lds) - kSplitRbStart, kSplitRbStart, V + kPad - 4 * KS);
     return;
   } else if constexpr (SPLIT) {
-    if (run) poly_round(0, fb.K, smp, -kPad, V + kPad - 4 * KS);
+    if (run) poly_round(rsA, smp, -kPad, V + kPad - 4 * KS);
     return;
   }
-  if (run) poly_round(0, fw.ka, smp, -kPad, min(V, kSA * T) + kPad - 4 * KS);
+  if (run) poly_round(rsA, smp, -kPad, min(V, kSA * T) + kPad - 4 * KS);
+  if constexpr (EARLY_TILES) request_tiles(rsB);
   RSMP_STAMP(6)
   __syncthreads();
   {
@@ -459,7 +477,7 @@
   }
   __syncthreads();
   if (tail_in_b) store_tail(reinterpret_cast<const double2 *>(lds), kSB0 * T);
-  if (run && fw.ka < fb.K) poly_round(fw.ka, fb.K, reinterpret_cast<const double2 *>(lds) - kSB0 * T, kSB0 * T, V + kPad - 4 * KS);
+  if (run) poly_round(rsB, reinterpret_cast<const double2 *>(lds) - kSB0 * T, kSB0 * T, V + kPad - 4 * KS);
   RSMP_STAMP(5)
 #ifdef RSMP_STAMPS_BUILD
   if (stamping && tid == 0) atomicAdd(a.stamps + 7, 1ull);
@@ -567,6 +585,7 @@
 
 hipError_t launch_fused_split(int omode, const FusedArgs &a, const FastIo &io, hipStream_t st, const char **kname)
 {
+  if (!a.blk || !a.wst) return hipErrorInvalidValue;
   if (a.d.two) {
     if (a.d.nsub != 1 || a.d.Vs != a.d.V || a.d.Pref != 4096 || a.d.V <= kSplitVsMax || a.d.V > 8192 || (a.d.V & 1)) return hipErrorInvalidValue;
   } else if (a.d.Vs > kSplitVsMax) return hipErrorInvalidValue;
@@ -608,26 +627,21 @@
   for (int i = 0; i < 13; ++i) head[i] = h[i];
   size_t n = 0;
   if (fb.cnt <= 0) return 0;
+  const WalkStart ws = fused_walk_start(fb, ngrp, pl);
   for (int round = 0; round < 2; ++round) {
-    const int kb = round ? fw.ka : 0, ke = round ? fb.K : fw.ka;
-    if (ke <= kb) continue;
-    const WalkRound wr = walk_round(fw, fb.K, kb, ke, ngrp);
-    const int cnt = walk_round_cnt(fb, fw, ke, pl);
+    const WalkStartRound &r = ws.r[round];
+    const int kb = r.kb, cnt = r.cnt;
     for (int wave = 0; wave < 4; ++wave) {
-      const int t0 = (wr.nt * wave) >> 2, t1 = (wr.nt * (wave + 1)) >> 2;
-      if (t0 >= t1) continue;
-      int g, c;
-      walk_seek(wr, t0, g, c);
-      int pc = 4 * c + walk_p0(fw, g), pend = walk_p0(fw, g) + 4 * walk_ncs(fw, fb.K, kb, ke, g);
-      for (int left = t1 - t0; left > 0; --left) {
+      int g = r.w[wave].g, pc = r.w[wave].pc, pend = r.w[wave].pend, p0 = pc & 3;
+      for (int left = r.w[wave].n; left > 0; --left) {
         for (int lane = 0; lane < 64; ++lane) {
           const int hi = lane >> 4, bq = (lane >> 2) & 3, jq = lane & 3, rloc = 4 * bq + hi;
           const long long a0 = p.at0 + (long long)(16 * g + 4 * bq) * step;
-          const int li = walk_lane_li(fb, kb, hi, jq, step) + int(a0 / pl) + pc * step;
-          const int ib = walk_lane_ib(fb, kb, jq, rloc, pl) + 16 * g + pc * pl;
+          const int li = walk_lane_li(fb.base_li, kb, hi, jq, step) + int(a0 / pl) + pc * step;
+          const int ib = walk_lane_ib(fb.irel_lo, kb, jq, rloc, pl) + 16 * g + pc * pl;
           if (n < cap) {
             int *o = slots + 7 * n;
-            o[0] = round, o[1] = g, o[2] = (pc - walk_p0(fw, g)) >> 2, o[3] = lane, o[4] = ib;
+            o[0] = round, o[1] = g, o[2] = (pc - p0) >> 2, o[3] = lane, o[4] = ib;
             o[5] = ib >= 0 && ib < cnt && 16 * g + rloc < pl;
             o[6] = li;
           }
@@ -635,14 +649,21 @@
         }
         if (pc + 4 == pend) {
           ++g;
-          pc = walk_p0(fw, g);
-          pend = pc + 4 * walk_ncs(fw, fb.K, kb, ke, g);
+          walk_next_group(r, g, p0, pend);
+          pc = p0;
         } else
           pc += 4;
       }
     }
   }
   return n;
+}
+
+void fused_walk_start_host(const FusedPrepArgs &p, int k, int *out56)
+{
+  static_assert(sizeof(WalkStart) == 56 * sizeof(int), "WalkStart as 56 ints");
+  const WalkStart ws = fused_walk_start(fused_block_info(p, k), (p.polyL + 15) >> 4, p.polyL);
+  memcpy(out56, &ws, sizeof ws);
 }
 
 bool fused_fast_supported(int log2n, int log2p, int ksteps)
@@ -659,6 +680,7 @@
 
 hipError_t launch_fused_fast(int log2p, const FusedArgs &a, const FastIo &io, hipStream_t st, const char **kname)
 {
+  if (!a.blk || !a.wst) return hipErrorInvalidValue;
   RSMP_FAST_CASE(11, 7) RSMP_FAST_CASE(12, 7) RSMP_FAST_CASE(11, 8) RSMP_FAST_CASE(12, 8)
   return hipErrorInvalidValue;
 }
diff --git a/foo_dsp_resampler_amd/csrc/kernels.hpp b/foo_dsp_resampler_amd/csrc/kernels.hpp
--- a/foo_dsp_resampler_amd/csrc/kernels.hpp
+++ b/foo_dsp_resampler_amd/csrc/kernels.hpp
@@ -174,8 +174,8 @@
   g = gb + dg;
   c = t - tb - dg * n;
 }
-__host__ __device__ inline int walk_lane_li(const FusedBlock &fb, int kb, int hi, int jq, int step) { return fb.base_li + hi + (kb + jq) * step; }
-__host__ __device__ inline int walk_lane_ib(const FusedBlock &fb, int kb, int jq, int rloc, int pl) { return (kb + jq) * pl + rloc - fb.irel_lo; }
+__host__ __device__ inline int walk_lane_li(int base_li, int kb, int hi, int jq, int step) { return base_li + hi + (kb + jq) * step; }
+__host__ __device__ inline int walk_lane_ib(int irel_lo, int kb, int jq, int rloc, int pl) { return (kb + jq) * pl + rloc - irel_lo; }
 __host__ __device__ inline int walk_round_cnt(const FusedBlock &fb, const FusedWalk &w, int ke, int pl)
 {
   const int irel_hi = fb.irel_lo + fb.cnt, e = (ke + (w.g_lo > 0 ? 1 : 0)) * pl;
@@ -266,6 +266,61 @@
   }
   return fb;
 }
+struct WalkStartWave { int n, g, pc, pend; };
+struct WalkStartRound {
+  int kb, ke, cnt;
+  int b1, b2;
+  int p0[3], pend[3];
+  int pad;
+  WalkStartWave w[4];
+};
+struct alignas(16) WalkStart { WalkStartRound r[2]; };
+static_assert(sizeof(WalkStartRound) == 112 && sizeof(WalkStart) == 224, "WalkStart: fixed layout (the kernels read it as dwords)");
+__host__ __device__ inline void fused_walk_start_round(const FusedBlock &fb, int ngrp, int pl, int round, WalkStartRound &r)
+{
+  const FusedWalk fw = fused_walk(fb, ngrp);
+  const int kb = round ? fw.ka : 0, ke = round ? fb.K : fw.ka;
+  const bool have = fb.cnt > 0 && ke > kb;
+  WalkRound wr = {0, 0, 0, 0, 0, 0, 0, 0};
+  if (have) wr = walk_round(fw, fb.K, kb, ke, ngrp);
+  r.kb = have ? kb : 0;
+  r.ke = have ? ke : 0;
+  r.cnt = have ? walk_round_cnt(fb, fw, ke, pl) : 0;
+  r.b1 = wr.b1;
+  r.b2 = wr.b2;
+  r.pad = 0;
+  const int gs[3] = {0, wr.b1, wr.b2};
+#pragma unroll
+  for (int i = 0; i < 3; ++i) {
+    const int p0 = walk_p0(fw, gs[i]);
+    r.p0[i] = have ? p0 : 0;
+    r.pend[i] = have ? p0 + 4 * walk_ncs(fw, fb.K, kb, ke, gs[i]) : 0;
+  }
+#pragma unroll
+  for (int wave = 0; wave < 4; ++wave) {
+    const int t0 = (wr.nt * wave) >> 2, t1 = (wr.nt * (wave + 1)) >> 2;
+    WalkStartWave e = {0, 0, 0, 0};
+    if (t0 < t1) {
+      int g, c;
+      walk_seek(wr, t0, g, c);
+      const int p0 = walk_p0(fw, g);
+      e = WalkStartWave{t1 - t0, g, 4 * c + p0, p0 + 4 * walk_ncs(fw, fb.K, kb, ke, g)};
+    }
+    r.w[wave] = e;
+  }
+}
+__host__ __device__ inline WalkStart fused_walk_start(const FusedBlock &fb, int ngrp, int pl)
+{
+  WalkStart s;
+  fused_walk_start_round(fb, ngrp, pl, 0, s.r[0]);
+  fused_walk_start_round(fb, ngrp, pl, 1, s.r[1]);
+  return s;
+}
+__host__ __device__ inline void walk_next_group(const WalkStartRound &r, int gnext, int &p0, int &pend)
+{
+  if (gnext == r.b2) p0 = r.p0[2], pend = r.pend[2];
+  else if (gnext == r.b1) p0 = r.p0[1], pend = r.pend[1];
+}
 constexpr int kFusedMaxBlocks = 1024;
 
 struct FusedArgs {
@@ -283,11 +338,11 @@
   int kper;
   const double *cfm;
   int NGRP, KS;
-  int reserved = 0;
   unsigned long long *stamps;
   const FusedBlock *blk;
   const int *qtab;
   const double2 *cfm2;
+  const WalkStart *wst = nullptr;
 };
 
 struct FastIo {
@@ -345,8 +400,9 @@
 hipError_t launch_seam(const AnyView &out, const FusedArgs &a, hipStream_t st);
 bool fused_shape_supported(int log2n, int log2p, int n, int span, int max_seam_outputs);
 bool fused_mfma_supported(int log2n, int log2p, int ksteps);
-hipError_t launch_fused_prep(const FusedPrepArgs &p, FusedBlock *out, hipStream_t st);
+hipError_t launch_fused_prep(const FusedPrepArgs &p, FusedBlock *out, hipStream_t st, WalkStart *wst = nullptr);
 size_t fused_walk_enumerate(const FusedPrepArgs &p, int k, long long *head, int *slots, size_t cap);
+void fused_walk_start_host(const FusedPrepArgs &p, int k, int *out56);
 
 struct PolyMfArgs {
   const double *cfm;
diff --git a/foo_dsp_resampler_amd/ratelib.py b/foo_dsp_resampler_amd/ratelib.py
--- a/foo_dsp_resampler_amd/ratelib.py
+++ b/foo_dsp_resampler_amd/ratelib.py
@@ -11,7 +11,7 @@
     "init_ratelib", "close_ratelib", "RR_open", "RR_flow", "RR_push", "RR_pull", "RR_drain", "RR_close", "RR_strerror",
     "RRX_open_batch", "RRX_open_batch_on", "RRX_device", "RRX_push_device", "RRX_pull_device", "RRX_flow_device", "RRX_push_strided", "RRX_pull_strided",
     "RRX_set_stream", "RRX_sync", "RRX_profile", "RRX_profile_read", "RRX_profile_report", "RRX_debug_fail_alloc",
-    "RRX_debug_tile_walk",
+    "RRX_debug_tile_walk", "RRX_debug_walk_start",
     "RRX_open_batch_fmt", "RRX_format", "RRX_push_double", "RRX_pull_double", "RRX_flow_double", "RRX_push_device_double",
     "RRX_pull_device_double", "RRX_flow_device_double",
     "RRX_push_samples", "RRX_pull_samples", "RRX_flow_samples", "RRX_push_device_samples", "RRX_pull_device_samples",
@@ -37,6 +37,19 @@
 class WalkGeom(C.Structure):
     _fields_ = [("at0", C.c_longlong), ("b_offset", C.c_longlong), ("B0", C.c_longlong)] + [
         (k, C.c_int) for k in ("V", "polyL", "step", "n", "KS", "qb_min", "qb_max", "two_round", "ra_end", "rb_start", "nsub", "Vs")]
+
+
+class WalkStartWave(C.Structure):
+    _fields_ = [(k, C.c_int) for k in ("n", "g", "pc", "pend")]
+
+
+class WalkStartRound(C.Structure):
+    _fields_ = [(k, C.c_int) for k in ("kb", "ke", "cnt", "b1", "b2")] + [("p0", C.c_int * 3), ("pend", C.c_int * 3), ("pad", C.c_int),
+                                                                         ("wave", WalkStartWave * 4)]
+
+
+class WalkStart(C.Structure):
+    _fields_ = [("round", WalkStartRound * 2)]
 
 
 class RRError(RuntimeError):
@@ -134,6 +147,8 @@
         if hasattr(L, "RRX_debug_tile_walk"):
             L.RRX_debug_tile_walk.argtypes = [P(WalkGeom), C.c_int, P(C.c_longlong), vp, sz]
             L.RRX_debug_tile_walk.restype = C.c_longlong
+        if hasattr(L, "RRX_debug_walk_start"):
+            L.RRX_debug_walk_start.argtypes = [P(WalkGeom), C.c_int, P(WalkStart)]
         for n in ("RRX_isamp_max", "RRX_available"):
             getattr(L, n).argtypes = [vp]
             getattr(L, n).restype = sz
diff --git a/include/ratelib_amd.h b/include/ratelib_amd.h
--- a/include/ratelib_amd.h
+++ b/include/ratelib_amd.h
@@ -35,6 +35,14 @@
   int V, polyL, step, n, KS, qb_min, qb_max, two_round, ra_end, rb_start, nsub, Vs;
 } RRX_walk_geom;
 long long RRX_debug_tile_walk(const RRX_walk_geom *geom, int k, long long *head, int *slots, size_t cap);
+
+typedef struct RRX_walk_start {
+  struct {
+    int kb, ke, cnt, b1, b2, p0[3], pend[3], pad;
+    struct { int n, g, pc, pend; } wave[4];
+  } round[2];
+} RRX_walk_start;
+int RRX_debug_walk_start(const RRX_walk_geom *geom, int k, RRX_walk_start *out);
 
 #define RRX_FMT_FLOAT  0
 #define RRX_FMT_DOUBLE 1
```

Result: faster. 126,500 Msamples/s, median of 6 (+1.3%).
